# microsoft/tf2-gnn

Measured on AMD Instinct MI355X. Metric: edges/sec (fwd+bwd) RGCN H=320 L=4, PPI-shaped batch, 1/2/4/8 MI355X, higher is better.
Workload: dtype f32; 1 GPU; rmat30k: V=30000 E=900000 per GPU (one batch per rank, replicas) edge_types=4 D=320 H=320 layers=4 RGCN (PPI_RGCN.json stack settings), step = edge bucketing of the next batch (2nd stream, overlapped) + forward (training mode) + f...

## Files before the change

include/tfgnn.h:

```cpp
#ifndef TFGNN_H
#define TFGNN_H

#include <stddef.h>
#include <stdint.h>

#ifdef __cplusplus
extern "C" {
#endif

typedef enum {
  TFGNN_OK = 0,
  TFGNN_ERR_INVALID_ARGUMENT = -1,
  TFGNN_ERR_OUT_OF_RANGE = -2,
  TFGNN_ERR_HIP = -3,
  TFGNN_ERR_UNSUPPORTED = -4
} tfgnn_status;

typedef enum {
  TFGNN_ACT_NONE = 0,
  TFGNN_ACT_RELU = 1,
  TFGNN_ACT_TANH = 2,
  TFGNN_ACT_LEAKY_RELU = 3,
  TFGNN_ACT_ELU = 4,
  TFGNN_ACT_SELU = 5,
// ... 286 lines not shown
                        const float* d_fixed_inv_scale, void* stream);
int tfgnn_sp_split_cols(const float* d_src, int64_t ld, int64_t K, int64_t N, void* d_sp, int64_t ld_sp_bytes,
                        float* d_inv_scale, void* stream);
int tfgnn_sp_gemm_nt(int64_t M, int64_t N, int64_t K, const void* d_A_sp, int64_t lda_bytes, const float* d_a_inv_scale,
                     int a_scale_block, const void* d_B_sp, int64_t ldb_bytes, const float* d_b_inv_scale, float* d_C,
                     int64_t ldc, const float* d_bias, int act, int accumulate, const float* d_mul, int64_t ld_mul,
                     int act_of_saved, const float* d_saved, int64_t ld_saved, void* stream);
int tfgnn_sp_gemm_nt_sp(int64_t M, int64_t N, int64_t K, const void* d_A_sp, int64_t lda_bytes, const float* d_a_inv_scale,
                        int a_scale_block, const void* d_B_sp, int64_t ldb_bytes, const float* d_b_inv_scale, float* d_C,
                        int64_t ldc, const float* d_bias, int act, const float* d_mul, int64_t ld_mul, int act_of_saved,
                        const float* d_saved, int64_t ld_saved, void* d_out_sp, int64_t ld_out_sp_bytes,
                        float* d_out_inv_scale, void* stream);
int tfgnn_sp_gemm_nt_rows(int64_t M, int64_t N, int64_t K, const void* d_A_sp, int64_t lda_bytes, const float* d_a_inv_scale,
                          int a_scale_block, const int32_t* d_a_rows, const void* d_B_sp, int64_t ldb_bytes, const float* d_b_inv_scale,
                          float* d_C, int64_t ldc, const float* d_bias, int act, int accumulate, const float* d_mul, int64_t ld_mul,
                          int act_of_saved, const float* d_saved, int64_t ld_saved, float saved_scale, void* d_out_sp,
                          int64_t ld_out_sp_bytes, float* d_out_inv_scale, float dropout_rate, uint64_t dropout_seed,
                          const uint8_t* d_tile_kmask, const int32_t* d_row_map, void* stream);

int tfgnn_sp_gemm_nt_grouped(int64_t M, int64_t N, int64_t K, const void* d_A_sp, int64_t lda_bytes, const float* d_a_inv_scale,
                             int a_scale_block, const int32_t* d_a_rows, int64_t a_src_rows, const int32_t* d_tile_table,
                             int64_t num_tiles, int num_groups, const void* d_B_sp, int64_t ldb_bytes, int64_t b_group_stride_bytes,
                             const float* d_b_inv_scale, int64_t b_scale_group_stride, float* d_C, int64_t ldc, const float* d_bias,
                             int act, const float* d_mul, int64_t ld_mul, int act_of_saved, const float* d_saved, int64_t ld_saved,
                             void* d_out_sp, int64_t ld_out_sp_bytes, float* d_out_inv_scale, void* stream);
int tfgnn_sp_gather_rows(const void* d_src_sp, int64_t ld_src_bytes, const float* d_src_inv_scale, int scales_per_row,
                         const int32_t* d_index, int64_t rows, int64_t src_rows, int64_t cols, void* d_dst_sp, int64_t ld_dst_bytes,
                         float* d_dst_inv_scale, void* stream);

size_t tfgnn_sp_gemm_tn_wide_workspace_bytes(int64_t M, int64_t N, int64_t K, int64_t a_total_cols, int a_scale_block);
int tfgnn_sp_gemm_tn_wide(int64_t M, int64_t N, int64_t K, const void* d_A_sp, int64_t lda_bytes, int64_t a_first_col,
                          const float* d_a_inv_scale, int64_t a_total_cols, int a_scale_block, const void* d_B_sp,
                          int64_t ldb_bytes, int64_t b_first_col, const float* d_b_inv_scale, float* d_C, int64_t group_rows,
                          int64_t stride_group, int64_t stride_row, int64_t stride_col, int accumulate, void* d_workspace,
                          size_t workspace_bytes, void* stream);

size_t tfgnn_sp_gemm_tn_grouped_workspace_bytes(int64_t M, int64_t N, int64_t a_total_cols, int a_scale_block, int num_splits);
int tfgnn_sp_gemm_tn_grouped(int64_t M, int64_t N, const void* d_A_sp, int64_t lda_bytes, const float* d_a_inv_scale,
                             int64_t a_total_cols, int a_scale_block, const void* d_B_sp, int64_t ldb_bytes, const float* d_b_inv_scale,
                             int num_groups, const int32_t* d_group_split_offsets, int num_splits, const int32_t* d_split_table,
                             float* d_C, int64_t c_group_stride, int64_t stride_row, int64_t stride_col, void* d_workspace,
                             size_t workspace_bytes, void* stream);

int tfgnn_sp_gemm_nt_set_splitk_workspace(void* d_workspace, size_t bytes);
int tfgnn_sp_gemm_nt_splitk_status(int enable, int* timed_out, int64_t* split_launches);

int tfgnn_sp_gemm_nt_dropout(int64_t M, int64_t N, int64_t K, const void* d_A_sp, int64_t lda_bytes, const float* d_a_inv_scale,
                             int a_scale_block, const void* d_B_sp, int64_t ldb_bytes, const float* d_b_inv_scale, float* d_C,
                             int64_t ldc, const float* d_bias, int act, int accumulate, const float* d_mul, int64_t ld_mul,
                             int act_of_saved, const float* d_saved, int64_t ld_saved, float saved_scale, void* d_out_sp,
                             int64_t ld_out_sp_bytes, float* d_out_inv_scale, float dropout_rate, uint64_t dropout_seed,
                             const uint8_t* d_tile_kmask, const int32_t* d_row_map, void* stream);

typedef struct tfgnn_aux_job {
  int kind;
  unsigned num_blocks;
  unsigned char payload[248];
} tfgnn_aux_job;
int tfgnn_aux_launch(const tfgnn_aux_job* jobs, int num_jobs, void* stream);
int tfgnn_sp_split_rows_job(const float* d_src, int64_t ld, int64_t seg_len, int64_t seg_stride, int64_t rows, int64_t cols,
                            int scale_block, void* d_sp, int64_t ld_sp_bytes, float* d_inv_scale,
                            const float* d_fixed_inv_scale, tfgnn_aux_job* job);
int tfgnn_sp_split_cols_job(const float* d_src, int64_t ld, int64_t K, int64_t N, void* d_sp, int64_t ld_sp_bytes,
                            float* d_inv_scale, tfgnn_aux_job* job);
size_t tfgnn_sp_split_cols_two_pass_bytes(int64_t K, int64_t N);
int tfgnn_sp_split_cols_jobs(const float* d_src, int64_t ld, int64_t K, int64_t N, void* d_sp, int64_t ld_sp_bytes,
                             float* d_inv_scale, float* d_colmax_workspace, size_t workspace_bytes, tfgnn_aux_job* maxima_job,
                             tfgnn_aux_job* split_job);
int tfgnn_graph_gather_reduce_sp_deferred(const tfgnn_graph* graph, int view, const int32_t* d_col_override,
                                          const float* d_edge_weight, const float* d_row_scale, const float* d_in,
                                          int64_t ld_in, int width, void* d_out_sp, int64_t ld_out_sp_bytes,
                                          float* d_inv_scale, const float* d_fixed_inv_scale, void* d_workspace,
                                          size_t workspace_bytes, tfgnn_aux_job* combine_job, void* stream);

size_t tfgnn_sp_gemm_tn_workspace_bytes(int64_t M, int64_t N, int64_t K, int64_t a_total_cols, int a_scale_block);
int tfgnn_sp_spread_flag(int reset);
int tfgnn_sp_guard_repair(int on);
int tfgnn_sp_repair_stats(int64_t* out2, int reset);
int tfgnn_sp_gemm_tn(int64_t M, int64_t N, int64_t K, const void* d_A_sp, int64_t lda_bytes, int64_t a_first_col,
                     const float* d_a_inv_scale, int64_t a_total_cols, int a_scale_block, const void* d_B_sp,
                     int64_t ldb_bytes, int64_t b_first_col, const float* d_b_inv_scale, float* d_C, int64_t group_rows,
                     int64_t stride_group, int64_t stride_row, int64_t stride_col, int accumulate, void* d_workspace,
                     size_t workspace_bytes, void* stream);

int tfgnn_absmax(const float* d_x, int64_t n, float scale, float* d_out, void* stream);
int tfgnn_sp_inv_scale_from_bound(const float* d_bound, float* d_inv_scale, void* stream);

int tfgnn_graph_gather_dot_supported(int width, int ew_heads);
int tfgnn_graph_gather_reduce_dot(const tfgnn_graph* g, int view, const float* d_edge_weight, int ew_heads, const float* d_in,
                                  int64_t ld_in, int width, float* d_out, int64_t ld_out, const float* d_dot_rows, int64_t ld_dot,
                                  const int32_t* d_dot_pos, float* d_dot_out, void* d_workspace, size_t workspace_bytes,
                                  void* stream);

int tfgnn_graph_gather_reduce_sp(const tfgnn_graph* graph, int view, const int32_t* d_col_override,
                                 const float* d_edge_weight, const float* d_row_scale, const float* d_in, int64_t ld_in,
                                 int width, void* d_out_sp, int64_t ld_out_sp_bytes, float* d_inv_scale,
                                 const float* d_fixed_inv_scale, void* d_workspace, size_t workspace_bytes, void* stream);

int tfgnn_transpose_batched(const float* d_src, int64_t batch, int64_t rows, int64_t cols, float* d_dst,
                            void* stream);

size_t tfgnn_task_metrics_workspace_bytes(void);
int tfgnn_sigmoid_ce_metrics(const float* d_logits, int64_t ld_logits, const float* d_labels, int64_t ld_labels,
                             int64_t V, int64_t C, float* d_metrics, int64_t* d_counts, float* d_dlogits,
                             void* d_workspace, size_t workspace_bytes, void* stream);
int tfgnn_regression_metrics(const float* d_pred, const float* d_target, int64_t G, float* d_metrics,
                             float* d_dpred, void* d_workspace, size_t workspace_bytes, void* stream);
int tfgnn_binary_ce_metrics(const float* d_logits, const float* d_target, int64_t G, float* d_prob, float* d_metrics,
                            int64_t* d_counts, float* d_dlogits, void* d_workspace, size_t workspace_bytes,
                            void* stream);

size_t tfgnn_softmax_ce_workspace_bytes(void);
int tfgnn_softmax_ce_metrics(const float* d_logits, int64_t ld_logits, const float* d_labels, int64_t ld_labels,
                             const float* d_weights, int64_t ld_weights, int64_t V, int64_t C, float* d_metrics,
                             int64_t* d_counts, float* d_dlogits, int64_t ld_dlogits, int32_t* d_pred,
                             void* d_workspace, size_t workspace_bytes, void* stream);

size_t tfgnn_distmult_ce_workspace_bytes(void);
int tfgnn_distmult_ce_metrics(const float* d_H, int64_t ld_H, const float* d_R, const int32_t* d_triples, const float* d_labels,
                              int64_t ld_labels, const float* d_weights, int64_t ld_weights, int64_t V, int64_t T, int64_t N,
                              int64_t D, float* d_metrics, int64_t* d_counts, float* d_scores, float* d_gscore,
                              void* d_workspace, size_t workspace_bytes, void* stream);
size_t tfgnn_distmult_backward_workspace_bytes(int64_t N, int64_t D);
int tfgnn_distmult_backward(const float* d_H, int64_t ld_H, const float* d_R, const int32_t* d_triples, const float* d_gscore,
                            const int32_t* d_node_offsets, const int32_t* d_node_entries, const int32_t* d_rel_offsets,
                            const int32_t* d_rel_order, int64_t V, int64_t T, int64_t N, int64_t D, float* d_dH, int64_t ld_dH,
                            int accumulate, float* d_dR, void* d_workspace, size_t workspace_bytes, void* stream);
size_t tfgnn_distmult_rank_workspace_bytes(int64_t Q);
int tfgnn_distmult_rank(const float* d_H, int64_t ld_H, const float* d_R, const int32_t* d_queries, int64_t Q, int side,
                        const int32_t* d_filter_offsets, const int32_t* d_filter_ids, int64_t V, int64_t T, int64_t D,
                        int32_t* d_greater, int32_t* d_equal, void* d_workspace, size_t workspace_bytes, void* stream);
int tfgnn_link_launch_counts(int64_t* out_counts, int n);

typedef enum {
  TFGNN_MP_AGGREGATE_FIRST = 0
} tfgnn_mp_kind;

typedef struct tfgnn_mp_forward_args {
  size_t struct_size;
  int kind;
  const tfgnn_graph* graph;
  int view;
  const float* x;
  int64_t ldx;
  int in_dim, hidden_dim;
  const float* row_scale;
  const float* w;
  void* wt_sp;
  int64_t ld_wt_sp_bytes;
  float* wt_inv_scale;
  void* agg_sp;
  float* agg_inv_scale;
  const float* bias;
  int act;
  float dropout_rate;
  uint64_t dropout_seed;
  const uint8_t* tile_kmask;
  const int32_t* row_map;
  float* out;
  int64_t ld_out;
  void* out_sp;
  int64_t ld_out_sp_bytes;
  float* out_inv_scale;
  void* workspace;
  size_t workspace_bytes;
} tfgnn_mp_forward_args;
// ... 217 lines not shown
```

tf2_gnn_amd/_lib.py:

```python
from __future__ import annotations

import ctypes
from ctypes import POINTER, c_char_p, c_float, c_int, c_int32, c_int64, c_size_t, c_void_p
from pathlib import Path

LIB_PATH = Path(__file__).resolve().parent / "libtfgnn.so"

_SIGNATURES = [
    ("tfgnn_last_error", c_char_p, []),
    ("tfgnn_version", c_char_p, []),
    ("tfgnn_abi_version", c_int, []),
    ("tfgnn_gemm_gathered_supported", c_int, [c_int64, c_int64, c_int64, c_int64, c_int64]),
    ("tfgnn_launch_counts", c_int, [POINTER(c_int64), c_int]),
    ("tfgnn_sp_spread_flag", c_int, [c_int]),
    ("tfgnn_sp_guard_repair", c_int, [c_int]),
    ("tfgnn_sp_repair_stats", c_int, [POINTER(c_int64), c_int]),
    (
        "tfgnn_graph_create",
        c_int,
        [c_int, c_int64, POINTER(c_void_p), POINTER(c_int64), c_void_p, POINTER(c_void_p)],
    ),
    ("tfgnn_graph_destroy", c_int, [c_void_p]),
    (
        "tfgnn_graph_create_async",
# ... 215 lines not shown
         c_void_p, c_int64, c_int64, c_int64, c_void_p, c_size_t, c_void_p],
    ),
    ("tfgnn_sp_gemm_tn_wide_workspace_bytes", c_size_t, [c_int64, c_int64, c_int64, c_int64, c_int]),
    (
        "tfgnn_sp_gemm_tn_wide",
        c_int,
        [c_int64, c_int64, c_int64, c_void_p, c_int64, c_int64, c_void_p, c_int64, c_int, c_void_p, c_int64, c_int64, c_void_p,
         c_void_p, c_int64, c_int64, c_int64, c_int64, c_int, c_void_p, c_size_t, c_void_p],
    ),
    (
        "tfgnn_sp_gemm_tn",
        c_int,
        [c_int64, c_int64, c_int64, c_void_p, c_int64, c_int64, c_void_p, c_int64, c_int, c_void_p, c_int64, c_int64, c_void_p,
         c_void_p, c_int64, c_int64, c_int64, c_int64, c_int, c_void_p, c_size_t, c_void_p],
    ),
    ("tfgnn_absmax", c_int, [c_void_p, c_int64, c_float, c_void_p, c_void_p]),
    ("tfgnn_sp_inv_scale_from_bound", c_int, [c_void_p, c_void_p, c_void_p]),
    ("tfgnn_sp_bytes", c_size_t, [c_int64, c_int64]),
    (
        "tfgnn_sp_split_rows",
        c_int,
        [c_void_p, c_int64, c_int64, c_int64, c_int64, c_int64, c_int, c_void_p, c_int64, c_void_p, c_void_p, c_void_p],
    ),
    ("tfgnn_sp_split_cols", c_int, [c_void_p, c_int64, c_int64, c_int64, c_void_p, c_int64, c_void_p, c_void_p]),
    (
        "tfgnn_sp_gemm_nt",
        c_int,
        [c_int64, c_int64, c_int64, c_void_p, c_int64, c_void_p, c_int, c_void_p, c_int64, c_void_p, c_void_p, c_int64,
         c_void_p, c_int, c_int, c_void_p, c_int64, c_int, c_void_p, c_int64, c_void_p],
    ),
    (
        "tfgnn_sp_gemm_nt_sp",
        c_int,
        [c_int64, c_int64, c_int64, c_void_p, c_int64, c_void_p, c_int, c_void_p, c_int64, c_void_p, c_void_p, c_int64,
         c_void_p, c_int, c_void_p, c_int64, c_int, c_void_p, c_int64, c_void_p, c_int64, c_void_p, c_void_p],
    ),
    ("tfgnn_aux_launch", c_int, [c_void_p, c_int, c_void_p]),
    (
        "tfgnn_sp_split_rows_job",
        c_int,
        [c_void_p, c_int64, c_int64, c_int64, c_int64, c_int64, c_int, c_void_p, c_int64, c_void_p, c_void_p, c_void_p],
    ),
    ("tfgnn_sp_split_cols_job", c_int, [c_void_p, c_int64, c_int64, c_int64, c_void_p, c_int64, c_void_p, c_void_p]),
    ("tfgnn_sp_split_cols_two_pass_bytes", c_size_t, [c_int64, c_int64]),
    ("tfgnn_sp_split_cols_jobs", c_int, [c_void_p, c_int64, c_int64, c_int64, c_void_p, c_int64, c_void_p, c_void_p, c_size_t, c_void_p,
                                         c_void_p]),
    (
        "tfgnn_graph_gather_reduce_sp_deferred",
        c_int,
        [c_void_p, c_int, c_void_p, c_void_p, c_void_p, c_void_p, c_int64, c_int, c_void_p, c_int64, c_void_p, c_void_p, c_void_p,
         c_size_t, c_void_p, c_void_p],
    ),
    (
        "tfgnn_sp_gemm_nt_dropout",
        c_int,
        [c_int64, c_int64, c_int64, c_void_p, c_int64, c_void_p, c_int, c_void_p, c_int64, c_void_p, c_void_p, c_int64,
         c_void_p, c_int, c_int, c_void_p, c_int64, c_int, c_void_p, c_int64, c_float, c_void_p, c_int64, c_void_p, c_float,
         ctypes.c_uint64, c_void_p, c_void_p, c_void_p],
    ),
    (
        "tfgnn_sp_gemm_nt_grouped",
        c_int,
        [c_int64, c_int64, c_int64, c_void_p, c_int64, c_void_p, c_int, c_void_p, c_int64, c_void_p, c_int64, c_int, c_void_p, c_int64,
         c_int64, c_void_p, c_int64, c_void_p, c_int64, c_void_p, c_int, c_void_p, c_int64, c_int, c_void_p, c_int64, c_void_p, c_int64,
         c_void_p, c_void_p],
    ),
    ("tfgnn_sp_gather_rows", c_int, [c_void_p, c_int64, c_void_p, c_int, c_void_p, c_int64, c_int64, c_int64, c_void_p, c_int64,
                                     c_void_p, c_void_p]),
    (
        "tfgnn_sp_gemm_nt_rows",
        c_int,
        [c_int64, c_int64, c_int64, c_void_p, c_int64, c_void_p, c_int, c_void_p, c_void_p, c_int64, c_void_p, c_void_p, c_int64,
         c_void_p, c_int, c_int, c_void_p, c_int64, c_int, c_void_p, c_int64, c_float, c_void_p, c_int64, c_void_p, c_float,
         ctypes.c_uint64, c_void_p, c_void_p, c_void_p],
    ),
]

_SIGNATURES += [
    ("tfgnn_mp_forward", c_int, [c_void_p, c_void_p]),
    ("tfgnn_mp_backward", c_int, [c_void_p, c_void_p]),
]

_SIGNATURES += [
    ("tfgnn_pool_workspace_bytes", c_size_t, [c_int64, c_int64, c_int, c_int, c_int]),
    ("tfgnn_pool_forward", c_int, [c_void_p, c_void_p]),
    ("tfgnn_pool_backward", c_int, [c_void_p, c_void_p]),
    ("tfgnn_pool_launch_counts", c_int, [POINTER(c_int64), c_int]),
]
POOL_SOFTMAX, POOL_SIGMOID, POOL_NONE, POOL_AVERAGE = range(4)
POOL_CHUNK_NODES = 128

_SIGNATURES += [
    ("tfgnn_optimizer_workspace_bytes", c_size_t, [c_void_p, c_int, c_int]),
    ("tfgnn_optimizer_apply", c_int, [c_void_p, c_int, c_void_p, c_void_p]),
    ("tfgnn_optimizer_iterations_get", c_int, [c_void_p, c_void_p, c_void_p]),
    ("tfgnn_optimizer_iterations_set", c_int, [c_void_p, c_int64, c_void_p]),
    ("tfgnn_optimizer_launch_count", c_int64, []),
]

_SIGNATURES += [
    ("tfgnn_batch_assemble", c_int, [c_void_p, c_void_p]),
    ("tfgnn_batch_assemble_launch_counts", c_int, [POINTER(c_int64), c_int]),
]
BATCH_MAX_EDGE_TYPES = 48
BATCH_MAX_COLUMNS = 8
BATCH_MAX_NODE_COLUMNS = 4

_SIGNATURES += [
    ("tfgnn_distmult_ce_workspace_bytes", c_size_t, []),
    (
        "tfgnn_distmult_ce_metrics",
        c_int,
        [c_void_p, c_int64, c_void_p, c_void_p, c_void_p, c_int64, c_void_p, c_int64, c_int64, c_int64, c_int64, c_int64, c_void_p,
         c_void_p, c_void_p, c_void_p, c_void_p, c_size_t, c_void_p],
    ),
    ("tfgnn_distmult_backward_workspace_bytes", c_size_t, [c_int64, c_int64]),
    (
        "tfgnn_distmult_backward",
        c_int,
        [c_void_p, c_int64, c_void_p, c_void_p, c_void_p, c_void_p, c_void_p, c_void_p, c_void_p, c_int64, c_int64, c_int64, c_int64,
         c_void_p, c_int64, c_int, c_void_p, c_void_p, c_size_t, c_void_p],
    ),
    ("tfgnn_distmult_rank_workspace_bytes", c_size_t, [c_int64]),
    (
        "tfgnn_distmult_rank",
        c_int,
        [c_void_p, c_int64, c_void_p, c_void_p, c_int64, c_int, c_void_p, c_void_p, c_int64, c_int64, c_int64, c_void_p, c_void_p,
         c_void_p, c_size_t, c_void_p],
    ),
    ("tfgnn_link_launch_counts", c_int, [POINTER(c_int64), c_int]),
]
LINK_CHUNK = 256

_SIGNATURES += [
    ("tfgnn_neighbor_sample_workspace_bytes", c_size_t, [c_int64, c_int, c_int64]),
    ("tfgnn_neighbor_sample", c_int, [c_void_p, c_void_p]),
    ("tfgnn_gather_node_rows", c_int, [c_void_p, c_void_p]),
    ("tfgnn_sample_launch_counts", c_int, [POINTER(c_int64), c_int]),
]
SAMPLE_MAX_HOPS = 8
SAMPLE_META_STATUS, SAMPLE_META_NODES, SAMPLE_META_EDGES = 0, 1, 2
SAMPLE_NODE_OVERFLOW, SAMPLE_EDGE_OVERFLOW, SAMPLE_REPEATED_SEED, SAMPLE_BAD_SEED, SAMPLE_BAD_STORE = 1, 2, 4, 8, 16


def sample_meta_words(num_edge_types: int, num_hops: int) -> int:
    return 2 + num_edge_types + num_hops + 2


EXPORTED_SYMBOLS = [s[0] for s in _SIGNATURES]
ABI_VERSION = 5


class AuxJob(ctypes.Structure):

    _fields_ = [("kind", c_int), ("num_blocks", ctypes.c_uint), ("payload", ctypes.c_ubyte * 248)]


class MpForwardArgs(ctypes.Structure):

    _fields_ = [
        ("struct_size", ctypes.c_size_t), ("kind", c_int), ("graph", c_void_p), ("view", c_int), ("x", c_void_p), ("ldx", c_int64),
        ("in_dim", c_int), ("hidden_dim", c_int), ("row_scale", c_void_p), ("w", c_void_p), ("wt_sp", c_void_p),
        ("ld_wt_sp_bytes", c_int64), ("wt_inv_scale", c_void_p), ("agg_sp", c_void_p), ("agg_inv_scale", c_void_p), ("bias", c_void_p),
        ("act", c_int), ("dropout_rate", ctypes.c_float), ("dropout_seed", ctypes.c_uint64), ("tile_kmask", c_void_p),
        ("row_map", c_void_p), ("out", c_void_p), ("ld_out", c_int64), ("out_sp", c_void_p), ("ld_out_sp_bytes", c_int64),
        ("out_inv_scale", c_void_p), ("workspace", c_void_p), ("workspace_bytes", ctypes.c_size_t),
    ]


class MpBackwardArgs(ctypes.Structure):

    _fields_ = [
        ("struct_size", ctypes.c_size_t), ("kind", c_int), ("graph", c_void_p), ("d_pre", c_void_p), ("ld_d_pre", c_int64),
        ("in_dim", c_int), ("hidden_dim", c_int), ("edge_weight", c_void_p), ("w", c_void_p), ("wh_sp", c_void_p),
        ("ld_wh_sp_bytes", c_int64), ("wh_inv_scale", c_void_p), ("g_sp", c_void_p), ("g_inv_scale", c_void_p), ("dx", c_void_p),
        ("ld_dx", c_int64), ("accumulate", c_int), ("mul", c_void_p), ("ld_mul", c_int64), ("act_of_saved", c_int), ("saved", c_void_p),
        ("ld_saved", c_int64), ("saved_scale", ctypes.c_float), ("dropout_rate", ctypes.c_float), ("dropout_seed", ctypes.c_uint64),
        ("dx_sp", c_void_p), ("ld_dx_sp_bytes", c_int64), ("dx_inv_scale", c_void_p), ("tile_kmask", c_void_p), ("a_rows", c_void_p),
        ("row_map", c_void_p), ("dw", c_void_p), ("x_sp", c_void_p), ("ld_x_sp_bytes", c_int64), ("x_inv_scale", c_void_p),
        ("tn_workspace", c_void_p), ("tn_workspace_bytes", ctypes.c_size_t), ("workspace", c_void_p),
        ("workspace_bytes", ctypes.c_size_t),
    ]


class PoolForwardArgs(ctypes.Structure):

    _fields_ = [
        ("struct_size", ctypes.c_size_t), ("kind", c_int), ("V", c_int64), ("G", c_int64), ("GD", c_int), ("heads", c_int),
        ("ptr", c_void_p), ("T", c_void_p), ("ldT", c_int64), ("S", c_void_p), ("ldS", c_int64), ("lo", c_float), ("hi", c_float),
        ("out", c_void_p), ("w", c_void_p), ("ldw", c_int64), ("workspace", c_void_p), ("workspace_bytes", ctypes.c_size_t),
    ]


class PoolBackwardArgs(ctypes.Structure):

    _fields_ = [
        ("struct_size", ctypes.c_size_t), ("kind", c_int), ("V", c_int64), ("G", c_int64), ("GD", c_int), ("heads", c_int),
        ("ptr", c_void_p), ("ids", c_void_p), ("dOut", c_void_p), ("T", c_void_p), ("ldT", c_int64), ("w", c_void_p),
        ("ldw", c_int64), ("lo", c_float), ("hi", c_float), ("dT", c_void_p), ("lddT", c_int64), ("dS", c_void_p),
        ("lddS", c_int64), ("workspace", c_void_p), ("workspace_bytes", ctypes.c_size_t),
    ]


class BatchAssembleArgs(ctypes.Structure):

    _fields_ = [
        ("struct_size", ctypes.c_size_t), ("num_edge_types", c_int), ("num_columns", c_int), ("num_graphs", c_int64),
        ("store_nodes", c_int64), ("feature_dim", c_int64), ("node_ptr", c_void_p), ("features", c_void_p), ("edge_ptr", c_void_p),
        ("edges", c_void_p), ("columns", c_void_p), ("order_len", c_int64), ("order", c_void_p), ("pos_node_ptr", c_void_p),
        ("pos_edge_ptr", c_void_p), ("p0", c_int64), ("p1", c_int64), ("num_nodes", c_int64), ("num_edges", c_void_p),
        ("node_features", c_void_p), ("node_to_graph_map", c_void_p), ("adjacency_lists", c_void_p), ("column_out", c_void_p),
        ("bad_flag", c_void_p), ("num_node_columns", c_int), ("node_column_widths", c_void_p), ("node_columns", c_void_p),
        ("node_column_out", c_void_p),
    ]


class NeighborSampleArgs(ctypes.Structure):

    _fields_ = [
        ("struct_size", ctypes.c_size_t), ("num_edge_types", c_int), ("num_hops", c_int), ("num_nodes", c_int64),
        ("in_ptr", c_void_p), ("in_src", c_void_p), ("store_edges", c_void_p), ("fanouts", c_void_p), ("seed", ctypes.c_uint64),
        ("num_seeds", c_int64), ("seeds", c_void_p), ("node_capacity", c_int64), ("edge_capacity", c_void_p), ("nodes", c_void_p),
        ("adjacency_lists", c_void_p), ("meta", c_void_p), ("workspace", c_void_p), ("workspace_bytes", ctypes.c_size_t),
    ]


class GatherNodeRowsArgs(ctypes.Structure):

    _fields_ = [
        ("struct_size", ctypes.c_size_t), ("store_nodes", c_int64), ("num_rows", c_int64), ("num_seeds", c_int64), ("nodes", c_void_p),
        ("feature_dim", c_int64), ("features", c_void_p), ("node_features", c_void_p), ("num_node_columns", c_int),
        ("node_column_widths", c_void_p), ("node_columns", c_void_p), ("node_column_out", c_void_p), ("seed_only", c_void_p),
        ("bad_flag", c_void_p),
    ]


class OptConfig(ctypes.Structure):

# ... 48 lines not shown
```

tf2_gnn_amd/csrc/gemm_sp.hip:

```cpp
#include <algorithm>
#include <cstdlib>

#include <type_traits>

#include "aux_jobs.hpp"
#include "common.hpp"
#include "gemm_sp.hpp"
#include "sp16.hpp"
#include "tn_repair.hpp"

namespace tfgnn {

template <int I, int N, class F>
__device__ __forceinline__ void static_for(F&& f) {
  if constexpr (I < N) {
    f(std::integral_constant<int, I>{});
    static_for<I + 1, N>(f);
  }
}

typedef _Float16 half8 __attribute__((ext_vector_type(8)));
typedef _Float16 half2v __attribute__((ext_vector_type(2)));
typedef float floatx16 __attribute__((ext_vector_type(16)));
typedef unsigned int uint4v __attribute__((ext_vector_type(4)));
typedef unsigned int uint2v __attribute__((ext_vector_type(2)));
typedef __attribute__((address_space(3))) void lds_void;

constexpr int SP_BM = 128;
constexpr int SP_NT = 256;

struct SpArgs {
  int64_t M, N, K;
  const uint8_t* A;
  int64_t lda;
  const float* a_inv;
  int64_t a_inv_ld;
  int a_nblk;
  int a_blk_steps;
  const uint8_t* B;
  int64_t ldb;
  const float* b_inv;
  float* C;
  int64_t ldc;
  const float* bias;
  int act;
  int accumulate;
  const float* mul;
  int64_t ld_mul;
  const float* saved;
  int64_t ld_saved;
  int dact;
  unsigned n_tiles;
  uint8_t* out_sp;
  int64_t ld_out_sp;
  float* out_inv;
  int drop_on;
  int64_t drop_ld;
  DropoutKey drop;
  float saved_scale;
  const uint8_t* tile_kmask;
  const int32_t* row_map;
  const int32_t* a_rows;
  int64_t a_src_rows;
  const int32_t* tile_table;
  int64_t group_stride_b;
  int64_t group_stride_scale;
  int ksplit;
  float* ws_partial;
  unsigned* ws_flags;
  int* ws_timeout;
  unsigned xcd_per, xcd_total;
};

__global__ void __launch_bounds__(256) sp_split_rows_kernel(const float* __restrict__ src, int64_t ld, int64_t seg_len,
                                                            int64_t seg_stride, int64_t R, int64_t C, int sb,
                                                            uint8_t* __restrict__ dst, int64_t ld_dst, float* __restrict__ inv,
                                                            const float* __restrict__ fixed_inv) {
  sp_split_rows_body(src, ld, seg_len, seg_stride, R, C, sb, dst, ld_dst, inv, fixed_inv, blockIdx.x);
}

template <int LPR>
__global__ void __launch_bounds__(256) sp_split_rows_narrow_kernel(const float* __restrict__ src, int64_t ld, int64_t R,
                                                                   uint8_t* __restrict__ dst, int64_t ld_dst, float* __restrict__ inv) {
  constexpr int RPB = 256 / LPR;
  const int sub = threadIdx.x % LPR;
  for (int64_t r = (int64_t)blockIdx.x * RPB + threadIdx.x / LPR; r < R; r += (int64_t)gridDim.x * RPB) {
    const float4 v = *reinterpret_cast<const float4*>(src + r * ld + sub * 4);
    float mx = fmaxf(fmaxf(fabsf(v.x), fabsf(v.y)), fmaxf(fabsf(v.z), fabsf(v.w)));
#pragma unroll
    for (int o = LPR / 2; o; o >>= 1) mx = fmaxf(mx, __shfl_xor(mx, o, 64));
    float iv;
    const float sc = sp_scale_for_max(mx, &iv);
    if (inv && sub == 0) inv[r] = iv;
    sp_store4(dst + r * ld_dst, sub * 4, v, sc);
  }
}

__global__ void __launch_bounds__(256) sp_absmax_kernel(const float* __restrict__ x, int64_t n, float scale, float* out) {
  float mx = 0.f;
  const int64_t n4 = n >> 2;
  for (int64_t i = (int64_t)blockIdx.x * blockDim.x + threadIdx.x; i < n4; i += (int64_t)gridDim.x * blockDim.x) {
    const float4 v = reinterpret_cast<const float4*>(x)[i];
    mx = fmaxf(mx, fmaxf(fmaxf(fabsf(v.x), fabsf(v.y)), fmaxf(fabsf(v.z), fabsf(v.w))));
  }
  if (blockIdx.x == 0 && threadIdx.x < (n & 3)) mx = fmaxf(mx, fabsf(x[(n4 << 2) + threadIdx.x]));
#pragma unroll
  for (int o = 32; o; o >>= 1) mx = fmaxf(mx, __shfl_xor(mx, o, 64));
  __shared__ float wmax[4];
  if ((threadIdx.x & 63) == 0) wmax[threadIdx.x >> 6] = mx;
  __syncthreads();
  if (threadIdx.x == 0)
    atomicMax(reinterpret_cast<unsigned*>(out), __float_as_uint(fmaxf(fmaxf(wmax[0], wmax[1]), fmaxf(wmax[2], wmax[3])) * scale));
}

__global__ void sp_inv_scale_kernel(const float* bound, float* inv) {
  float iv;
  (void)sp_scale_for_max(fabsf(bound[0]), &iv);
  inv[0] = iv;
}

__global__ void __launch_bounds__(256) sp_split_cols_kernel(const float* __restrict__ src, int64_t ld, int64_t K, int64_t N,
                                                            uint8_t* __restrict__ dst, int64_t ld_dst, float* __restrict__ inv) {
  sp_split_cols_body(src, ld, K, N, dst, ld_dst, inv, blockIdx.x, blockIdx.y, gridDim.y);
}

template <int TNW>
constexpr int sp_nt_tm = TNW == 5 ? 1 : 2;

template <int TNW, int TM = 2>
struct SpGeo {
  static constexpr int BN = 64 * TNW;
  static constexpr int ROWS = SP_BM + BN;
  static constexpr int STG = ROWS * 64;
  static constexpr int NW = 8 / TM;
  static constexpr int NT = 64 * NW;
  static constexpr int ND_A = 8 / NW;
  static constexpr int ND_B = 4 * TNW / NW;
  static constexpr int ND = ND_A + ND_B;
  static constexpr bool PAIR = TM == 1;
  static constexpr bool SHARED = (4 * TNW) % NW != 0;
  static constexpr int NI = PAIR ? 2 * ND + (SHARED ? 1 : 0) : ND;
  static_assert(!SHARED || (PAIR && 4 * TNW - NW * ND_B == NW / 2), "left-over units go to wave pairs");
  static constexpr int PATCH_ROWS = 16 * TM;
  static constexpr int PATCH_LD = 32 * TNW + 4;
  static constexpr int NST_MAX = TNW == 2 ? 4 : 6;
  static constexpr int NST = (163840 / STG) < NST_MAX ? (163840 / STG) : NST_MAX;
  static constexpr int UNR = NST % 2 == 0 ? NST : 2 * NST;
  static constexpr int VMW = PAIR ? NI : (NST - 3) * ND;
  static constexpr int LDS_BYTES = NST * STG;
  static_assert(NST >= 4 && VMW < 64, "ring depth");
  static_assert(!PAIR || NST % 2 == 1, "pair issue fills the ring NST - 1 steps ahead, two steps at a time");
  static_assert(NW * PATCH_ROWS * PATCH_LD * 4 + TM * NW * 32 * 4 <= LDS_BYTES, "epilogue patch and row maxima must fit the ring");
};

template <int TNW, int TM>
struct SpLoop {
// ... 99 lines not shown
    if constexpr (I < N) {
      read_one<I, SET, ST>();
      read_all<I + 1, N, SET, ST>();
    }
  }

  const float* a_inv;
  int a_nblk, a_blk_steps;
  int64_t a_row[TM];
  float a_rmax[TM];
  half2v afac[TM];
  template <int SET>
  __device__ __forceinline__ void scale_frags(int step) {
    asm volatile("s_waitcnt lgkmcnt(0)" ::: "memory");
    const int lstep = step + (int)step0;
    if (lstep % a_blk_steps == 0 || step == 0) {
      const int q = step < nsteps ? lstep / a_blk_steps : 0;
      const int b = bsteps ? (int)((blkmap >> (4u * (unsigned)q)) & 15u) : q;
      if (step < nsteps && b < a_nblk) {
#pragma unroll
        for (int t = 0; t < TM; ++t) {
          const _Float16 f = (_Float16)(a_inv[a_row[t] * a_nblk + b] / a_rmax[t]);
          afac[t] = half2v{f, f};
        }
      }
    }
#pragma unroll
    for (int t = 0; t < TM; ++t)
#pragma unroll
      for (int p = 0; p < 2; ++p) {
        half2v* v = reinterpret_cast<half2v*>(&fa[SET][t][p]);
#pragma unroll
        for (int j = 0; j < 4; ++j) v[j] = v[j] * afac[t];
      }
  }

  static constexpr int NR = 2 * TM + 2 * TNW;
  static constexpr int NM = 3 * TM * TNW;
  static constexpr int DMA0 = NM - G::NI < NR ? NM - G::NI : NR;
  static_assert(DMA0 >= 0 && DMA0 + G::NI <= NM, "issue pattern");
  template <int S, int I, bool ABLK>
  __device__ __forceinline__ void step_items(int sbase) {
    if constexpr (I < NM) {
      mfma_one<I, (S & 1)>();
      if constexpr (I < NR) read_one<I, ((S + 1) & 1), ((S + 1) % G::NST)>();
      if constexpr (G::PAIR) {
        if constexpr ((S & 1) == 0 && I >= DMA0 && I < DMA0 + G::NI) dma_pair<I - DMA0, S>();
      } else {
        if constexpr (I >= DMA0 && I < DMA0 + G::NI) dma_one<I - DMA0, ((S + G::NST - 1) % G::NST)>(sbase + S + G::NST - 1);
      }
      if constexpr (ABLK && I == NM - 1) scale_frags<((S + 1) & 1)>(sbase + S + 1);
      step_items<S, I + 1, ABLK>(sbase);
    }
  }
  template <int S, bool ABLK>
  __device__ __forceinline__ void step(int sbase) {
    if constexpr (G::PAIR && (S & 1) == 0) pair_offsets(sbase + S);
    step_items<S, 0, ABLK>(sbase);
    asm volatile("s_waitcnt vmcnt(%0) lgkmcnt(0)" ::"n"(G::VMW) : "memory");
    __builtin_amdgcn_s_barrier();
  }
  template <int S, bool ABLK>
  __device__ __forceinline__ void steps(int sbase) {
    if constexpr (S < G::UNR) {
      if (sbase + S < nsteps) step<S, ABLK>(sbase);
      steps<S + 1, ABLK>(sbase);
    }
  }
  template <int J>
  __device__ __forceinline__ void dma_prologue() {
    if constexpr (G::PAIR) {
      if constexpr (2 * J < G::NST - 1) {
        pair_offsets(-(G::NST - 1) + 2 * J);
        dma_pair_all<0, (G::NST + 1 + 2 * J) % G::UNR>();
        dma_prologue<J + 1>();
      }
    } else if constexpr (J < G::NST - 1) {
      dma_all<0, G::ND, J>(J);
      dma_prologue<J + 1>();
    }
  }
};

template <int TNW, bool ABLK, bool GRAD, bool OUT_SP = false>
__global__ void __launch_bounds__((SpGeo<TNW, sp_nt_tm<TNW>>::NT), (TNW == 2 ? 2 : 1)) gemm_sp_nt_kernel(SpArgs g) {
  constexpr int TM = sp_nt_tm<TNW>;
  using G = SpGeo<TNW, TM>;
  constexpr int WR = 32 * TM;
  extern __shared__ __attribute__((aligned(16))) uint8_t lds[];
  const int tid = threadIdx.x;
  const int lane = tid & 63;
  const int wave = __builtin_amdgcn_readfirstlane(tid >> 6);
  const int wm = wave >> 1, wn = wave & 1;
  unsigned bid = blockIdx.x;
  if (g.xcd_per) {
    bid = (blockIdx.x & 7u) * g.xcd_per + (blockIdx.x >> 3);
    if (bid >= g.xcd_total) return;
  }
  int split = 0;
  int S = g.ksplit;
  if (S > 1) {
    const unsigned nt_all = gridDim.x / (unsigned)S;
    if (bid < nt_all * (unsigned)(S - 1)) {
      split = 1 + (int)(bid / nt_all);
      bid -= (unsigned)(split - 1) * nt_all;
    } else {
      bid -= nt_all * (unsigned)(S - 1);
    }
  }
  const unsigned tile_n = bid % g.n_tiles;
  const unsigned tile_m = bid / g.n_tiles;
  int64_t row0 = (int64_t)tile_m * SP_BM, m_end = g.M;
  int64_t grp = 0;
  if (g.tile_table) {
    const int32_t* e = g.tile_table + 4 * (int64_t)tile_m;
    row0 = __builtin_amdgcn_readfirstlane(e[0]);
    m_end = row0 + __builtin_amdgcn_readfirstlane(e[1]);
    grp = __builtin_amdgcn_readfirstlane(e[2]);
  }
  const int64_t col0 = (int64_t)tile_n * G::BN;
  int nsteps = (int)(g.K >> 4);
  unsigned blkmap = 0, bsteps = 0;
  if (g.tile_kmask) {
    unsigned m = __builtin_amdgcn_readfirstlane((int)g.tile_kmask[tile_m]) & ((1u << g.a_nblk) - 1u);
    if (!m) m = 1u;
    int n = 0;
    for (int b = 0; b < g.a_nblk; ++b)
      if (m & (1u << b)) blkmap |= (unsigned)b << (4 * n++);
    bsteps = (unsigned)g.a_blk_steps;
    nsteps = n * g.a_blk_steps;
  }
  unsigned step0 = 0;
  if (S > 1) {
    const int P = (int)(g.K >> 4);
    const int per = (P + S - 1) / S;
    const int p0 = split * per, p1 = p0 + per < P ? p0 + per : P;
    if (!bsteps) {
      step0 = (unsigned)p0;
      nsteps = p1 > p0 ? p1 - p0 : 0;
    } else {
      int first = -1, cnt = 0;
      const int nb = nsteps / (int)bsteps;
      for (int q = 0; q < nb; ++q) {
        const int b = (int)((blkmap >> (4u * (unsigned)q)) & 15u);
        const int lo = p0 > b * (int)bsteps ? p0 : b * (int)bsteps;
        const int hi = p1 < (b + 1) * (int)bsteps ? p1 : (b + 1) * (int)bsteps;
        if (hi > lo) {
          if (first < 0) first = q * (int)bsteps + (lo - b * (int)bsteps);
          cnt += hi - lo;
        }
      }
      step0 = first < 0 ? 0u : (unsigned)first;
      nsteps = cnt;
    }
  }

  const int64_t rows_a = m_end - row0 < SP_BM ? m_end - row0 : SP_BM;
  const int64_t rows_b = g.N - col0 < G::BN ? g.N - col0 : G::BN;
  auto make_rsrc = [](const uint8_t* p, int64_t bytes) {
    const uint64_t a = (uint64_t)(uintptr_t)p;
    return uint4v{(unsigned)__builtin_amdgcn_readfirstlane((int)(unsigned)a),
                  (unsigned)__builtin_amdgcn_readfirstlane((int)(unsigned)((a >> 32) & 0xffffu)),
                  (unsigned)__builtin_amdgcn_readfirstlane((int)bytes), 0x00020000u};
  };
  const uint4v rs_a = g.a_rows ? make_rsrc(g.A, g.a_src_rows * g.lda) : make_rsrc(g.A + row0 * g.lda, rows_a * g.lda);
  const uint4v rs_b = make_rsrc(g.B + grp * g.group_stride_b + col0 * g.ldb, rows_b * g.ldb);
  half8 r_fa[2][TM][2];
  half8 r_fb[2][TNW][2];
  floatx16 r_acc[TM][TNW];
  unsigned r_aa[G::NST][2], r_ba[G::NST][2], r_va[G::ND_A], r_vb[SpLoop<TNW, TM>::NVB];
  SpLoop<TNW, TM> L(r_fa, r_fb, r_acc, r_aa, r_ba, r_va, r_vb);
  L.rs_a = rs_a;
  L.rs_b = rs_b;
  const unsigned lds_base = (unsigned)(uintptr_t)(lds_void*)lds;
  L.m0_a = __builtin_amdgcn_readfirstlane(lds_base + wave * G::ND_A * 1024);
  L.m0_b = __builtin_amdgcn_readfirstlane(lds_base + wave * G::ND_B * 1024);
  L.m0_s = __builtin_amdgcn_readfirstlane(lds_base + SP_BM * 64 + (G::NW * G::ND_B + (wave >> 1)) * 1024);
  L.half_s = wave & 1;
  L.nsteps = nsteps;
  L.blkmap = blkmap;
  L.step0 = step0;
  L.bsteps = bsteps;
  L.brecip = bsteps ? (65536u + bsteps - 1u) / bsteps : 0u;
  const int drow = lane >> 2;
  const int dq = (lane & 3) ^ ((drow >> 2) & 3);
// ... 766 lines not shown
          fa[j] = 0.f;
          anz[j] = false;
          if (j < nb && k < krows) {
            const float ia = g.inv_a[(k0 + k) * g.a_nblk + blk_first + j];
            fa[j] = ia * fref[j];
            anz[j] = ia > 1.2e-38f;
            if (anz[j]) famax = fmaxf(famax, fa[j]);
          }
        }
        const bool bnz = k < krows && ib > 1.2e-38f;
        const float fbv = k < krows ? ib * frefb : 0.f;
        float fb2 = fbv, up = 1.f;
        if (bnz && famax > 0.f) {
          const unsigned ex = (__float_as_uint(famax * fbv) >> 23) & 0xffu;
          if (ex > 0u && ex <= 127u) {
            const unsigned tb = (127u - ex) >> 1;
            fb2 = __uint_as_float((127u - tb) << 23);
            up = fbv * __uint_as_float((127u + tb) << 23);
          }
        }
        ftab[(k >> 4) * FH + 64 + (k & 15)] = (_Float16)fb2;
        wide |= bnz && famax > 0.f && fb2 < 2.384185791015625e-07f;
#pragma unroll
        for (int j = 0; j < 4; ++j) {
          const float f = anz[j] ? fa[j] * up : 0.f;
          ftab[(k >> 4) * FH + j * 16 + (k & 15)] = (_Float16)f;
          wide |= anz[j] && bnz && f < 2.384185791015625e-07f;
        }
      } else {
#pragma unroll
        for (int j = 0; j < 4; ++j) {
          float f = 0.f, ia = 0.f;
          if (j < nb && k < krows) {
            ia = g.inv_a[(k0 + k) * g.a_nblk + blk_first + j];
            f = sp_row_holds(ia, ib) ? ia * ib * fref[j] : 0.f;
          }
          ftab[(k >> 4) * FH + j * 16 + (k & 15)] = (_Float16)f;
          wide |= sp_row_too_small(f, ia, ib);
        }
      }
    }
    if (g.spread_flag && __any(wide) && lane == 0) g.spread_flag[split * g.trip_stride] = 1;
  }
  L.wait_landed();
  __builtin_amdgcn_s_barrier();
  __builtin_amdgcn_sched_barrier(0);
  L.template load_factors<0>(0);
  L.template read_all<0, NR, 0, 0>();
  L.template scale_all<0, (BSC ? NR : 4), 0>();
  __builtin_amdgcn_sched_barrier(0);
  for (int s = 0; s < nsteps; s += G::UNR) L.template steps<0>(s);
  asm volatile("s_waitcnt vmcnt(0)\n\ts_nop 15\n\ts_nop 15" ::: "memory");
  __builtin_amdgcn_s_barrier();

  float* patch = reinterpret_cast<float*>(lds) + wave * 32 * G::PATCH_LD;
  float* __restrict__ part = g.partial + (int64_t)split * g.M * g.N;
  const int64_t wcol0 = col0 + wn * 32 * TNW;
  constexpr int C4 = 8 * TNW;
  constexpr int NIT = 32 * C4 / 64;
  auto store_tile = [&](auto t_c) {
    constexpr int t = decltype(t_c)::value;
#pragma unroll
    for (int c = 0; c < TNW; ++c)
#pragma unroll
      for (int r = 0; r < 16; ++r) {
        const int prow = (r & 3) + 8 * (r >> 2) + 4 * kg;
        patch[prow * G::PATCH_LD + c * 32 + fi] = L.acc[t][c][r];
      }
    asm volatile("s_waitcnt lgkmcnt(0)" ::: "memory");
    const int64_t wrow0 = row0 + wm * 64 + t * 32;
#pragma unroll
    for (int it = 0; it < NIT; ++it) {
      const int idx = lane + it * 64;
      const int pr = idx / C4, c4 = idx - pr * C4;
      const float4 v = *reinterpret_cast<const float4*>(patch + pr * G::PATCH_LD + c4 * 4);
      *reinterpret_cast<float4*>(part + (wrow0 + pr) * g.N + wcol0 + c4 * 4) = v;
    }
    asm volatile("s_waitcnt lgkmcnt(0)" ::: "memory");
  };
  store_tile(std::integral_constant<int, 0>{});
  store_tile(std::integral_constant<int, 1>{});
}

struct TnReduceArgs {
  const float* partial;
  int splits;
  int64_t M, N;
  const float* ref;
  int64_t a_col0;
  int a_sb;
  float* C;
  int64_t group_rows, stride_group, stride_row, stride_col;
  int accumulate;
  int64_t slab;
  int ref_ld;
};

__device__ __forceinline__ void sp_tn_reduce_body(const TnReduceArgs& a, unsigned block, unsigned nblocks) {
  const int64_t total = a.M * a.N;
  for (int64_t i = (int64_t)block * 256 + threadIdx.x; i < total; i += (int64_t)nblocks * 256) {
    const int64_t m = i / a.N, n = i - m * a.N;
    const int64_t blk = (a.a_col0 + m) / a.a_sb;
    float s = 0.f;
    int z = 0;
    if (a.ref_ld > 0) {
      for (; z + 8 <= a.splits; z += 8) {
        float v[8], r[8];
#pragma unroll
        for (int u = 0; u < 8; ++u) {
          v[u] = a.partial[(int64_t)(z + u) * a.slab + i];
          r[u] = a.ref[(int64_t)(z + u) * a.ref_ld + blk];
        }
#pragma unroll
        for (int u = 0; u < 8; ++u) s += v[u] * r[u];
      }
      for (; z < a.splits; ++z) s += a.partial[(int64_t)z * a.slab + i] * a.ref[(int64_t)z * a.ref_ld + blk];
    } else {
      for (; z + 8 <= a.splits; z += 8) {
        float v[8];
#pragma unroll
        for (int u = 0; u < 8; ++u) v[u] = a.partial[(int64_t)(z + u) * a.slab + i];
#pragma unroll
        for (int u = 0; u < 8; ++u) s += v[u];
      }
      for (; z < a.splits; ++z) s += a.partial[(int64_t)z * a.slab + i];
      s *= a.ref[blk];
    }
    const int64_t gi = m / a.group_rows, mi = m - gi * a.group_rows;
    float* dst = a.C + gi * a.stride_group + mi * a.stride_row + n * a.stride_col;
    *dst = a.accumulate ? *dst + s : s;
  }
}

__global__ void __launch_bounds__(256) sp_tn_reduce_kernel(TnReduceArgs a) { sp_tn_reduce_body(a, blockIdx.x, gridDim.x); }
__global__ void __launch_bounds__(256) sp_tn_reduce_grouped_kernel(TnReduceArgs a, const int32_t* __restrict__ split_off,
                                                                   int64_t c_group_stride) {
  const int gq = blockIdx.y;
  const int s0 = split_off[gq], s1 = split_off[gq + 1];
  a.partial += (int64_t)s0 * a.slab;
  a.ref += (int64_t)s0 * a.ref_ld;
  a.splits = s1 - s0;
  a.C += (int64_t)gq * c_group_stride;
  sp_tn_reduce_body(a, blockIdx.x, gridDim.x);
}

static int sp_tn_splits(int64_t M, int64_t N, int64_t K, int bn) {
  const int64_t tiles = (M / SP_BM) * (N / bn);
  const int64_t steps = (K + 15) / 16;
  int64_t splits = std::max<int64_t>(1, std::min<int64_t>(250 / std::max<int64_t>(tiles, 1), steps / 16));
  return (int)std::max<int64_t>(1, splits);
}

template <int TNW>
static void launch_sp_nt(const SpArgs& g_in, dim3 grid, hipStream_t s) {
  using G = SpGeo<TNW, sp_nt_tm<TNW>>;
  SpArgs g = g_in;
  g.xcd_per = g.xcd_total = 0;
  static const bool xcd_order = [] { const char* e = getenv("TFGNN_SP_NT_XCD"); return !(e && atoi(e) == 0); }();
  if (xcd_order && g.n_tiles > 1 && g.ksplit <= 1 && grid.y == 1 && grid.z == 1 && grid.x >= 16) {
    g.xcd_total = grid.x;
    g.xcd_per = (grid.x + 7u) / 8u;
    grid.x = g.xcd_per * 8u;
  }
  const bool ablk = g.a_inv && g.a_nblk > 1;
  const bool grad = g.mul || g.saved;
  count_launch(TFGNN_KFAM_SP_NT);
  using Kernel = void (*)(SpArgs);
  static const Kernel kernels[2][2][2] = {
      {{gemm_sp_nt_kernel<TNW, false, false, false>, gemm_sp_nt_kernel<TNW, false, false, true>},
       {gemm_sp_nt_kernel<TNW, false, true, false>, gemm_sp_nt_kernel<TNW, false, true, true>}},
      {{gemm_sp_nt_kernel<TNW, true, false, false>, gemm_sp_nt_kernel<TNW, true, false, true>},
       {gemm_sp_nt_kernel<TNW, true, true, false>, gemm_sp_nt_kernel<TNW, true, true, true>}}};
  static bool attr_set[2][2][2] = {};
  const bool out_sp = g.out_sp != nullptr;
  const Kernel kernel = kernels[ablk][grad][out_sp];
  if (!attr_set[ablk][grad][out_sp]) {
    (void)hipFuncSetAttribute((const void*)kernel, hipFuncAttributeMaxDynamicSharedMemorySize, G::LDS_BYTES);
    attr_set[ablk][grad][out_sp] = true;
  }
  hipLaunchKernelGGL(kernel, grid, dim3(G::NT), G::LDS_BYTES, s, g);
}

constexpr size_t kSplitkFlagBytes = 65536;
struct SplitkWorkspace {
  void* base = nullptr;
  size_t bytes = 0;
  bool enabled = true;
  long long split_launches = 0;
  long long timeouts = 0;
  int device = -1;
  hipStream_t last_stream = nullptr;
  bool used = false;
  int* timeout_host = nullptr;
  int* timeout_dev = nullptr;
};
static SplitkWorkspace g_splitk;

static bool stream_is_capturing(hipStream_t s) {
  hipStreamCaptureStatus st = hipStreamCaptureStatusNone;
  if (hipStreamIsCapturing(s, &st) != hipSuccess) {
    (void)hipGetLastError();
    return false;
  }
  return st != hipStreamCaptureStatusNone;
}

static int splitk_admit(hipStream_t s) {
  if (!(g_splitk.enabled && g_splitk.base)) return 0;
  if (g_splitk.timeout_host && __atomic_load_n(g_splitk.timeout_host, __ATOMIC_RELAXED)) {
    ++g_splitk.timeouts;
    __atomic_store_n(g_splitk.timeout_host, 0, __ATOMIC_RELAXED);
    (void)hipDeviceSynchronize();
    (void)hipMemset(g_splitk.base, 0, kSplitkFlagBytes);
    set_error("tfgnn_sp_gemm_nt: a reducer of an earlier K-split product gave up waiting for its producers - that product's "
              "result is incomplete; the workspace flags were cleared (tfgnn_sp_gemm_nt_splitk_status reports the count)");
    return -1;
  }
  int dev = -1;
  if (hipGetDevice(&dev) != hipSuccess || dev != g_splitk.device) {
    (void)hipGetLastError();
    return 0;
  }
  if (g_splitk.used && s != g_splitk.last_stream) {
    if (stream_is_capturing(g_splitk.last_stream)) return 0;
    if (!stream_is_capturing(s)) {
      if (hipStreamSynchronize(g_splitk.last_stream) != hipSuccess) {
        (void)hipGetLastError();
        return 0;
      }
    }
  }
  g_splitk.last_stream = s;
  g_splitk.used = true;
  return 1;
}

static int sp_colmax_parts(int64_t K) { return (int)std::max<int64_t>(1, std::min<int64_t>(256, K / 160)); }

static int sp_tile_width(int64_t N) { return N % 320 == 0 ? 320 : (N % 256 == 0 ? 256 : (N % 128 == 0 ? 128 : 0)); }

static int* g_spread_host = nullptr;
static int* g_spread_dev = nullptr;
static int* sp_spread_flag_device() {
  if (!g_spread_host) {
    int* h = nullptr;
    if (hipHostMalloc((void**)&h, 64, hipHostMallocMapped) != hipSuccess) {
      (void)hipGetLastError();
      return nullptr;
    }
    *h = 0;
    void* d = nullptr;
    if (hipHostGetDevicePointer(&d, h, 0) != hipSuccess) {
      (void)hipGetLastError();
      (void)hipHostFree(h);
      return nullptr;
    }
    g_spread_host = h;
    g_spread_dev = (int*)d;
  }
  return g_spread_dev;
}

constexpr int kSpTnMaxRanges = 512;
static_assert(kSpTnMaxRanges == kTnRepairGroupedMaxRanges, "the repair tail holds one trip word per K range of a launch");

struct TnLayout {
  size_t ref, ref_split, slabs, tail, total;
  int64_t f_ld;
};
static TnLayout sp_tn_layout(int64_t Mp, int64_t N, int64_t nblk, int64_t kpad, bool factor_pass, int64_t ranges, size_t tail_bytes) {
  TnLayout l;
  const int pass_floats = factor_pass ? 1 + SP_TN_MAXCHUNKS : 0;
  l.ref = factor_pass ? ((size_t)nblk * kpad * 2 + 255) & ~(size_t)255 : 0;
  l.ref_split = l.ref + (size_t)nblk * pass_floats * 4;
  l.slabs = l.ref + (((size_t)nblk * (pass_floats + kSpTnMaxRanges) * 4 + 255) & ~(size_t)255);
  l.tail = l.slabs + (size_t)ranges * (size_t)Mp * (size_t)N * 4;
  l.total = l.tail + tail_bytes;
  l.f_ld = factor_pass ? kpad : 0;
  return l;
}

enum class TnForm { FactorPass, OneFactor, TwoFactor };

template <int TNW, bool FIK, bool BSC>
static void launch_sp_tn_form(const SpTnArgs& g, dim3 grid, hipStream_t s) {
  constexpr int lds = SpGeoTN<TNW, FIK, BSC>::LDS_BYTES;
  [[maybe_unused]] static const hipError_t attr_set =
      hipFuncSetAttribute((const void*)gemm_sp_tn_kernel<TNW, FIK, BSC>, hipFuncAttributeMaxDynamicSharedMemorySize, lds);
  hipLaunchKernelGGL((gemm_sp_tn_kernel<TNW, FIK, BSC>), grid, dim3(SP_NT), lds, s, g);
}

template <int TNW>
static void launch_sp_tn(TnForm form, const SpTnArgs& g, dim3 grid, hipStream_t s) {
  count_launch(TFGNN_KFAM_SP_TN);
  if (form == TnForm::TwoFactor) launch_sp_tn_form<TNW, true, true>(g, grid, s);
  else if (form == TnForm::OneFactor) launch_sp_tn_form<TNW, true, false>(g, grid, s);
  else launch_sp_tn_form<TNW, false, false>(g, grid, s);
}

struct TnLaunch {
  int64_t M, N, K;
  const uint8_t *A, *B;
  int64_t lda, ldb;
  const float *inv_a, *inv_b;
  int a_sb, a_nblk;
  int64_t a_col0;
  int splits;
  int64_t k_chunk;
  const int32_t* split_table;
  TnForm form;
  uint8_t* ws;
  TnLayout lay;
  bool repair;
  int trip_stride;
  float* C;
  int64_t group_rows, stride_group, stride_row, stride_col;
  int accumulate;
  int num_groups;
  const int32_t* group_split_offsets;
  int64_t c_group_stride;
};

static int sp_tn_enqueue(const TnLaunch& t, hipStream_t s) {
  const int bn = sp_tile_width(t.N);
  const int64_t Mp = ceil_div(t.M, SP_BM) * SP_BM;
  const bool armed = t.repair && t.splits > 0, per_split = t.form != TnForm::FactorPass;
  float* ref = (float*)(t.ws + t.lay.ref);
  float* ref_split = (float*)(t.ws + t.lay.ref_split);
  int* guard_word = sp_spread_flag_device();
  if (armed) {
    guard_word = (int*)(t.ws + t.lay.tail);
    if (int rc = tn_repair_begin(guard_word, t.trip_stride ? kTnRepairGroupedTailBytes : sizeof(int), s)) return rc;
  }
  SpTnArgs g{};
  g.M = Mp; g.N = t.N; g.K = t.K;
  g.A = t.A; g.lda = t.lda;
  g.B = t.B; g.ldb = t.ldb;
  g.F = t.lay.f_ld ? (const _Float16*)t.ws : nullptr; g.f_ld = t.lay.f_ld;
  g.a_sb = t.a_sb; g.a_col0 = t.a_col0; g.a_nblk = t.a_nblk;
  g.inv_a = t.inv_a; g.inv_b = t.inv_b; g.ref_split = ref_split; g.spread_flag = guard_word;
  g.trip_stride = t.trip_stride;
  g.partial = (float*)(t.ws + t.lay.slabs);
  g.k_chunk = t.k_chunk;
  g.split_table = t.split_table;
  g.n_tiles = (unsigned)(t.N / bn);
  g.tiles = (unsigned)((Mp / SP_BM) * g.n_tiles);
  g.splits = (unsigned)t.splits;
  g.per_xcd = (g.tiles * g.splits + 7) / 8;
  if (t.form == TnForm::FactorPass) {
    const int fch = sp_tn_fchunks(t.K);
    float* slice_max = nullptr;
    if (fch > SP_TN_FCHUNKS) {
      slice_max = ref + t.a_nblk;
      hipLaunchKernelGGL(sp_tn_slice_max_kernel, dim3((unsigned)t.a_nblk * fch), dim3(1024), 0, s, t.inv_a, (int64_t)t.a_nblk, t.inv_b,
                         (int64_t)1, t.K, slice_max, fch);
    }
    hipLaunchKernelGGL(sp_tn_factors_kernel, dim3((unsigned)t.a_nblk * fch), dim3(1024), 0, s, t.inv_a, (int64_t)t.a_nblk, t.inv_b,
                       (int64_t)1, t.K, (_Float16*)t.ws, t.lay.f_ld, ref, guard_word, fch, (const float*)slice_max);
    TFGNN_LAUNCH_CHECK();
  }
  if (t.splits > 0) {
    const dim3 grid(8 * g.per_xcd);
    if (bn == 320) launch_sp_tn<5>(t.form, g, grid, s);
    else if (bn == 256) launch_sp_tn<4>(t.form, g, grid, s);
    else launch_sp_tn<2>(t.form, g, grid, s);
    TFGNN_LAUNCH_CHECK();
  }
  if (armed) {
    TnRepairArgs rp{};
    rp.M = t.M; rp.N = t.N; rp.K = t.K; rp.A = t.A; rp.lda = t.lda; rp.B = t.B; rp.ldb = t.ldb;
    rp.inv_a = t.inv_a; rp.inv_b = t.inv_b; rp.a_sb = t.a_sb; rp.a_col0 = t.a_col0; rp.a_nblk = t.a_nblk;
    rp.partial = g.partial; rp.slab = Mp * t.N; rp.splits = t.splits;
    rp.k_chunk = t.split_table ? 0 : t.k_chunk; rp.split_table = t.split_table;
    rp.ref = per_split ? ref_split : ref; rp.ref_per_split = per_split ? 1 : 0; rp.trip = guard_word;
    if (int rc = tn_repair_enqueue(rp, s)) return rc;
  }
  TnReduceArgs ra{};
  ra.partial = g.partial; ra.M = t.M; ra.N = t.N; ra.ref = per_split ? ref_split : ref; ra.a_col0 = t.a_col0; ra.a_sb = t.a_sb;
  ra.ref_ld = per_split ? t.a_nblk : 0;
  ra.splits = t.group_split_offsets ? 0 : t.splits;
  ra.C = t.C; ra.group_rows = t.group_rows; ra.stride_group = t.stride_group; ra.stride_row = t.stride_row; ra.stride_col = t.stride_col;
  ra.accumulate = t.accumulate; ra.slab = Mp * t.N;
  const int64_t rblocks = ceil_div(t.M * t.N, 256);
  if (t.group_split_offsets) {
    hipLaunchKernelGGL(sp_tn_reduce_grouped_kernel, dim3((unsigned)std::min<int64_t>(rblocks, 512), (unsigned)t.num_groups), dim3(256), 0, s,
                       ra, t.group_split_offsets, t.c_group_stride);
  } else {
    hipLaunchKernelGGL(sp_tn_reduce_kernel, dim3((unsigned)std::min<int64_t>(rblocks, 2048)), dim3(256), 0, s, ra);
  }
  TFGNN_LAUNCH_CHECK();
  return TFGNN_OK;
}

static int sp_tn_check_operands(const char* who, int64_t M, int64_t N, const void* d_A_sp, int64_t lda_bytes, int64_t a_first_col,
                                int64_t a_total_cols, int a_scale_block, const void* d_B_sp, int64_t ldb_bytes, int64_t b_first_col,
                                bool column_ranges) {
  if (!sp_tile_width(N) || M % 16 || a_scale_block < 32) {
    set_error("%s: M = %lld must be a multiple of 16, N = %lld of 128, scale blocks of A >= 32 columns", who, (long long)M, (long long)N);
    return TFGNN_ERR_UNSUPPORTED;
  }
  TFGNN_REQUIRE(lda_bytes % 64 == 0 && ldb_bytes % 64 == 0 && (uintptr_t)d_A_sp % 64 == 0 && (uintptr_t)d_B_sp % 64 == 0 &&
                    a_first_col % 16 == 0 && b_first_col % 16 == 0 && a_first_col >= 0 && b_first_col >= 0 &&
                    lda_bytes >= (a_first_col + M) * 4 && ldb_bytes >= (b_first_col + N) * 4 && a_total_cols >= a_first_col + M &&
                    a_total_cols % a_scale_block == 0,
                "%s: SP16 operands must be 64-byte aligned%s", who,
                column_ranges ? ", first columns multiples of 16, rows wide enough" : " with rows wide enough");
  return TFGNN_OK;
}

static int sp_tn_check_workspace(const char* who, const void* d_workspace, size_t workspace_bytes, size_t need) {
  TFGNN_REQUIRE(d_workspace && workspace_bytes >= need && (uintptr_t)d_workspace % 256 == 0,
                "%s: workspace too small or unaligned (need %zu bytes)", who, need);
  return TFGNN_OK;
}

struct NtShape {
  int bn;
  int a_scale_block;
  bool a_uniform;
  int64_t a_src_rows;
  int64_t group_stride_b;
  int drop_on;
  DropoutKey drop;
  int64_t tiles;
};

static int sp_nt_check(const NtCall& c, NtShape* d) {
  const int64_t M = c.M, N = c.N, K = c.K;
  TFGNN_REQUIRE(c.A && c.B && (c.C || c.out_sp), "tfgnn_sp_gemm_nt: null pointer");
  d->a_src_rows = (!c.a_rows || c.a_src_rows <= 0) ? M : c.a_src_rows;
  TFGNN_REQUIRE(!c.a_rows || d->a_src_rows * c.lda_bytes < (1ll << 32) - 65536, "tfgnn_sp_gemm_nt_rows: the operand read through a row index must be below 4 GB");
  TFGNN_REQUIRE(!c.tile_table || (c.num_tiles_m > 0 && c.num_groups >= 1 && !c.tile_kmask && !c.row_map),
                "tfgnn_sp_gemm_nt_grouped: a tile table needs its tile count and excludes the tile mask / row map");
  TFGNN_REQUIRE(c.dropout_rate >= 0.f && c.dropout_rate < 1.f, "tfgnn_sp_gemm_nt: dropout rate must be in [0, 1), got %f", (double)c.dropout_rate);
  TFGNN_REQUIRE(M > 0 && N > 0 && K > 0 && K % 16 == 0, "tfgnn_sp_gemm_nt: K must be a positive multiple of 16");
  d->bn = sp_tile_width(N);
  if (!d->bn) {
    set_error("tfgnn_sp_gemm_nt: N = %lld is not a multiple of 128", (long long)N);
    return TFGNN_ERR_UNSUPPORTED;
  }
  TFGNN_REQUIRE(c.lda_bytes % 64 == 0 && c.ldb_bytes % 64 == 0 && c.lda_bytes >= K * 4 && c.ldb_bytes >= K * 4 &&
                    (uintptr_t)c.A % 64 == 0 && (uintptr_t)c.B % 64 == 0,
                "tfgnn_sp_gemm_nt: SP16 operands must be 64-byte aligned with leading dimensions >= 4 K bytes");
  TFGNN_REQUIRE((!c.C || (c.ldc % 4 == 0 && (uintptr_t)c.C % 16 == 0)) && (!c.bias || (uintptr_t)c.bias % 16 == 0) &&
                    (!c.b_inv_scale || (uintptr_t)c.b_inv_scale % 16 == 0) && (!c.mul || (c.ld_mul % 4 == 0 && (uintptr_t)c.mul % 16 == 0)) &&
                    (!c.saved || (c.ld_saved % 4 == 0 && (uintptr_t)c.saved % 16 == 0)),
                "tfgnn_sp_gemm_nt: C / bias / scale / factor operands must be 16-byte aligned with ld %% 4 == 0");
  TFGNN_REQUIRE(128 * c.lda_bytes < (1ll << 31) && 320 * c.ldb_bytes < (1ll << 31), "tfgnn_sp_gemm_nt: K too large");
  d->a_uniform = c.a_scale_block < 0;
  d->a_scale_block = (c.a_scale_block <= 0 || c.a_scale_block >= K) ? (int)K : c.a_scale_block;
  TFGNN_REQUIRE(d->a_scale_block % 16 == 0 && K % d->a_scale_block == 0, "tfgnn_sp_gemm_nt: a_scale_block must divide K and be a multiple of 16");
  if (c.tile_kmask) {
    const int a_nblk = (int)(K / d->a_scale_block), a_blk_steps = d->a_scale_block / 16;
    TFGNN_REQUIRE(a_nblk >= 1 && a_nblk <= 8 && a_blk_steps <= 64 && a_blk_steps * a_nblk == (int)(K >> 4) && c.a_inv_scale &&
                      !d->a_uniform,
                  "tfgnn_sp_gemm_nt: the tile mask needs 1..8 scale blocks of A (of at most 1024 columns) that tile K");
  }
  d->group_stride_b = c.b_group_stride_bytes >= 0 ? c.b_group_stride_bytes : N * c.ldb_bytes;
  TFGNN_REQUIRE(d->group_stride_b % 64 == 0, "tfgnn_sp_gemm_nt_grouped: group stride of B must be a multiple of 64 bytes");
  d->drop_on = c.dropout_rate > 0.f ? (c.dropout_seed == ~0ull ? 2 : 1) : 0;
  if (d->drop_on == 2)
    TFGNN_REQUIRE(c.saved && c.act_of_saved == TFGNN_ACT_RELU, "tfgnn_sp_gemm_nt_dropout: the mask-from-saved form needs a relu saved tensor");
  d->drop = dropout_key(c.dropout_seed, c.dropout_rate);
  TFGNN_REQUIRE(c.dropout_rate <= 0.f || d->drop.epoch, "tfgnn_sp_gemm_nt_dropout: no device memory for this device's epoch word");
  if (c.out_sp) {
    TFGNN_REQUIRE(!c.accumulate && c.out_inv_scale, "tfgnn_sp_gemm_nt_sp: the split result needs no accumulation and an inverse-scale array");
    TFGNN_REQUIRE(c.ld_out_sp_bytes >= N * 4 && c.ld_out_sp_bytes % 64 == 0 && (uintptr_t)c.out_sp % 64 == 0,
                  "tfgnn_sp_gemm_nt_sp: SP16 result rows must be 64-byte aligned and at least 4 N bytes");
  }
  d->tiles = (c.tile_table ? c.num_tiles_m : ceil_div(M, SP_BM)) * (unsigned)(N / d->bn);
  TFGNN_REQUIRE(d->tiles <= 0x7fffffff, "tfgnn_sp_gemm_nt: too many tiles");
  return TFGNN_OK;
}

static SpArgs sp_nt_args(const NtCall& c, const NtShape& d) {
  SpArgs g{};
  g.M = c.M; g.N = c.N; g.K = c.K;
  g.A = (const uint8_t*)c.A; g.lda = c.lda_bytes; g.a_inv = c.a_inv_scale;
  g.a_nblk = (int)(c.K / d.a_scale_block);
  g.a_inv_ld = d.a_uniform ? 0 : g.a_nblk;
  g.a_blk_steps = d.a_scale_block / 16;
  g.B = (const uint8_t*)c.B; g.ldb = c.ldb_bytes; g.b_inv = c.b_inv_scale;
  g.C = c.C; g.ldc = c.ldc; g.bias = c.bias; g.act = c.act; g.accumulate = c.accumulate;
  g.mul = c.mul; g.ld_mul = c.ld_mul; g.saved = c.saved; g.ld_saved = c.ld_saved; g.dact = c.act_of_saved;
  g.saved_scale = c.saved_scale;
  g.tile_kmask = c.tile_kmask;
  g.row_map = c.row_map;
  g.a_rows = c.a_rows;
  g.a_src_rows = d.a_src_rows;
  g.tile_table = c.tile_table;
  g.group_stride_b = d.group_stride_b;
  g.group_stride_scale = c.b_scale_group_stride >= 0 ? c.b_scale_group_stride : c.N;
  g.drop_on = d.drop_on;
  g.drop_ld = c.N;
  g.drop = d.drop;
  g.n_tiles = (unsigned)(c.N / d.bn);
  if (c.out_sp) {
    g.out_sp = (uint8_t*)c.out_sp; g.ld_out_sp = c.ld_out_sp_bytes; g.out_inv = c.out_inv_scale;
  }
  g.ksplit = 1;
  return g;
}

constexpr int kSplitkMaxSplits = 4;
constexpr int64_t kSplitkMinSteps = 15;
constexpr int64_t kSplitkMaxWorkgroups = 232;
constexpr int64_t kSplitkMaxTiles = 112;

static int sp_nt_plan_splitk(SpArgs& g, const NtShape& d, hipStream_t s) {
  const int64_t steps = g.K >> 4;
  int S = (int)std::min<int64_t>(kSplitkMaxSplits, steps / kSplitkMinSteps);
  while (S > 1 && d.tiles * S > kSplitkMaxWorkgroups) --S;
  if (!(g_splitk.enabled && g_splitk.base && S > 1 && d.tiles <= kSplitkMaxTiles && !g.tile_table)) return TFGNN_OK;
  const size_t slab = (size_t)SP_BM * d.bn * 4;
  const size_t need = kSplitkFlagBytes + (size_t)d.tiles * (S - 1) * slab;
  const int admit = (need <= g_splitk.bytes && (size_t)d.tiles * (S - 1) * 4 <= kSplitkFlagBytes) ? splitk_admit(s) : 0;
  if (admit < 0) return TFGNN_ERR_HIP;
  if (admit > 0) {
    g.ksplit = S;
    ++g_splitk.split_launches;
    g.ws_flags = (unsigned*)g_splitk.base;
    g.ws_partial = (float*)((char*)g_splitk.base + kSplitkFlagBytes);
    g.ws_timeout = g_splitk.timeout_dev;
  }
  return TFGNN_OK;
}

int sp_nt_enqueue(const NtCall& c, hipStream_t s) {
  NtShape d;
  int rc = sp_nt_check(c, &d);
  if (rc) return rc;
  SpArgs g = sp_nt_args(c, d);
  rc = sp_nt_plan_splitk(g, d, s);
  if (rc) return rc;
  const dim3 grid((unsigned)(d.tiles * g.ksplit));
  if (d.bn == 320) launch_sp_nt<5>(g, grid, s);
  else if (d.bn == 256) launch_sp_nt<4>(g, grid, s);
  else launch_sp_nt<2>(g, grid, s);
  TFGNN_LAUNCH_CHECK();
  return TFGNN_OK;
}

}

using namespace tfgnn;

extern "C" {

size_t tfgnn_sp_bytes(int64_t rows, int64_t cols) { return (size_t)rows * (size_t)cols * 4; }

int tfgnn_sp_spread_flag(int reset) {
  if (!g_spread_host) return 0;
  const int v = __atomic_load_n(g_spread_host, __ATOMIC_RELAXED);
  if (reset) __atomic_store_n(g_spread_host, 0, __ATOMIC_RELAXED);
  return v;
}

int tfgnn_sp_split_rows(const float* d_src, int64_t ld, int64_t seg_len, int64_t seg_stride, int64_t rows, int64_t cols,
                        int scale_block, void* d_sp, int64_t ld_sp_bytes, float* d_inv_scale,
                        const float* d_fixed_inv_scale, void* stream) {
  TFGNN_REQUIRE(d_src && d_sp, "tfgnn_sp_split_rows: null pointer");
  TFGNN_REQUIRE(rows >= 0 && cols > 0 && cols % 16 == 0, "tfgnn_sp_split_rows: cols must be a positive multiple of 16");
  if (scale_block <= 0) scale_block = (int)cols;
  if (seg_len <= 0) { seg_len = cols; seg_stride = 0; }
  TFGNN_REQUIRE(scale_block % 16 == 0 && cols % scale_block == 0, "tfgnn_sp_split_rows: scale_block must divide cols and be a multiple of 16");
  TFGNN_REQUIRE(seg_len % 4 == 0 && cols % seg_len == 0 && ld % 4 == 0 && seg_stride % 4 == 0 && (uintptr_t)d_src % 16 == 0,
                "tfgnn_sp_split_rows: source must be 16-byte aligned with segment length / strides multiples of 4");
  TFGNN_REQUIRE(ld_sp_bytes >= cols * 4 && ld_sp_bytes % 64 == 0 && (uintptr_t)d_sp % 64 == 0, "tfgnn_sp_split_rows: bad SP16 leading dimension / alignment");
  if (rows == 0) return TFGNN_OK;
  if (!d_fixed_inv_scale && scale_block == cols && (seg_len <= 0 || seg_len >= cols) && rows >= 4096 &&
      (cols == 64 || cols == 128 || cols == 256)) {
    const unsigned rpb = (unsigned)(256 / (cols / 4));
    const unsigned grid = (unsigned)std::min<int64_t>(ceil_div(rows, rpb), 256 * 32);
    hipStream_t s = (hipStream_t)stream;
    if (cols == 64) hipLaunchKernelGGL(sp_split_rows_narrow_kernel<16>, dim3(grid), dim3(256), 0, s, d_src, ld, rows, (uint8_t*)d_sp, ld_sp_bytes, d_inv_scale);
    else if (cols == 128) hipLaunchKernelGGL(sp_split_rows_narrow_kernel<32>, dim3(grid), dim3(256), 0, s, d_src, ld, rows, (uint8_t*)d_sp, ld_sp_bytes, d_inv_scale);
    else hipLaunchKernelGGL(sp_split_rows_narrow_kernel<64>, dim3(grid), dim3(256), 0, s, d_src, ld, rows, (uint8_t*)d_sp, ld_sp_bytes, d_inv_scale);
    TFGNN_LAUNCH_CHECK();
    return TFGNN_OK;
  }
  const int64_t items = rows * (cols / scale_block);
  hipLaunchKernelGGL(sp_split_rows_kernel, dim3((unsigned)ceil_div(items, 4)), dim3(256), 0, (hipStream_t)stream, d_src, ld,
                     seg_len, seg_stride, rows, cols, scale_block, (uint8_t*)d_sp, ld_sp_bytes, d_inv_scale, d_fixed_inv_scale);
  TFGNN_LAUNCH_CHECK();
  return TFGNN_OK;
}

int tfgnn_sp_split_cols(const float* d_src, int64_t ld, int64_t K, int64_t N, void* d_sp, int64_t ld_sp_bytes,
                        float* d_inv_scale, void* stream) {
  TFGNN_REQUIRE(d_src && d_sp, "tfgnn_sp_split_cols: null pointer");
  TFGNN_REQUIRE(K > 0 && N > 0 && K % 16 == 0 && N % 4 == 0 && ld % 4 == 0 && (uintptr_t)d_src % 16 == 0,
                "tfgnn_sp_split_cols: K must be a multiple of 16, N and ld multiples of 4");
  TFGNN_REQUIRE(ld_sp_bytes >= K * 4 && ld_sp_bytes % 64 == 0 && (uintptr_t)d_sp % 64 == 0, "tfgnn_sp_split_cols: bad SP16 leading dimension / alignment");
  hipLaunchKernelGGL(sp_split_cols_kernel, dim3((unsigned)ceil_div(N, 16), (unsigned)std::max<int64_t>(1, std::min<int64_t>(8, K / 128))), dim3(256), 0, (hipStream_t)stream, d_src, ld, K, N,
                     (uint8_t*)d_sp, ld_sp_bytes, d_inv_scale);
  TFGNN_LAUNCH_CHECK();
  return TFGNN_OK;
}

int tfgnn_sp_gemm_nt_set_splitk_workspace(void* d_workspace, size_t bytes) {
  TFGNN_HIP_CHECK(hipDeviceSynchronize());
  if (!d_workspace || bytes <= kSplitkFlagBytes) {
    g_splitk.base = nullptr;
    g_splitk.bytes = 0;
    return TFGNN_OK;
  }
  TFGNN_REQUIRE((uintptr_t)d_workspace % 256 == 0, "tfgnn_sp_gemm_nt_set_splitk_workspace: the workspace must be 256-byte aligned");
  if (!g_splitk.timeout_host) {
    int* h = nullptr;
    void* d = nullptr;
    if (hipHostMalloc((void**)&h, 64, hipHostMallocMapped) == hipSuccess && hipHostGetDevicePointer(&d, h, 0) == hipSuccess) {
      *h = 0;
      g_splitk.timeout_host = h;
      g_splitk.timeout_dev = (int*)d;
    } else {
      (void)hipGetLastError();
    }
  }
  TFGNN_HIP_CHECK(hipMemset(d_workspace, 0, kSplitkFlagBytes));
  TFGNN_HIP_CHECK(hipGetDevice(&g_splitk.device));
  g_splitk.base = d_workspace;
// ... 47 lines not shown
                             int a_scale_block, const void* d_B_sp, int64_t ldb_bytes, const float* d_b_inv_scale, float* d_C,
                             int64_t ldc, const float* d_bias, int act, int accumulate, const float* d_mul, int64_t ld_mul,
                             int act_of_saved, const float* d_saved, int64_t ld_saved, float saved_scale, void* d_out_sp,
                             int64_t ld_out_sp_bytes, float* d_out_inv_scale, float dropout_rate, uint64_t dropout_seed,
                             const uint8_t* d_tile_kmask, const int32_t* d_row_map, void* stream) {
  NtCall c;
  c.M = M; c.N = N; c.K = K;
  c.A = d_A_sp; c.lda_bytes = lda_bytes; c.a_inv_scale = d_a_inv_scale; c.a_scale_block = a_scale_block;
  c.B = d_B_sp; c.ldb_bytes = ldb_bytes; c.b_inv_scale = d_b_inv_scale;
  c.C = d_C; c.ldc = ldc; c.accumulate = accumulate;
  c.out_sp = d_out_sp; c.ld_out_sp_bytes = ld_out_sp_bytes; c.out_inv_scale = d_out_inv_scale;
  c.bias = d_bias; c.act = act;
  c.mul = d_mul; c.ld_mul = ld_mul; c.act_of_saved = act_of_saved; c.saved = d_saved; c.ld_saved = ld_saved;
  c.saved_scale = saved_scale; c.dropout_rate = dropout_rate; c.dropout_seed = dropout_seed;
  c.tile_kmask = d_tile_kmask; c.row_map = d_row_map;
  return sp_nt_enqueue(c, (hipStream_t)stream);
}

int tfgnn_sp_gemm_nt_rows(int64_t M, int64_t N, int64_t K, const void* d_A_sp, int64_t lda_bytes, const float* d_a_inv_scale,
                          int a_scale_block, const int32_t* d_a_rows, const void* d_B_sp, int64_t ldb_bytes, const float* d_b_inv_scale,
                          float* d_C, int64_t ldc, const float* d_bias, int act, int accumulate, const float* d_mul, int64_t ld_mul,
                          int act_of_saved, const float* d_saved, int64_t ld_saved, float saved_scale, void* d_out_sp,
                          int64_t ld_out_sp_bytes, float* d_out_inv_scale, float dropout_rate, uint64_t dropout_seed,
                          const uint8_t* d_tile_kmask, const int32_t* d_row_map, void* stream) {
  NtCall c;
  c.M = M; c.N = N; c.K = K;
  c.A = d_A_sp; c.lda_bytes = lda_bytes; c.a_inv_scale = d_a_inv_scale; c.a_scale_block = a_scale_block; c.a_rows = d_a_rows;
  c.B = d_B_sp; c.ldb_bytes = ldb_bytes; c.b_inv_scale = d_b_inv_scale;
  c.C = d_C; c.ldc = ldc; c.accumulate = accumulate;
  c.out_sp = d_out_sp; c.ld_out_sp_bytes = ld_out_sp_bytes; c.out_inv_scale = d_out_inv_scale;
  c.bias = d_bias; c.act = act;
  c.mul = d_mul; c.ld_mul = ld_mul; c.act_of_saved = act_of_saved; c.saved = d_saved; c.ld_saved = ld_saved;
  c.saved_scale = saved_scale; c.dropout_rate = dropout_rate; c.dropout_seed = dropout_seed;
  c.tile_kmask = d_tile_kmask; c.row_map = d_row_map;
  return sp_nt_enqueue(c, (hipStream_t)stream);
}

int tfgnn_sp_gemm_nt_grouped(int64_t M, int64_t N, int64_t K, const void* d_A_sp, int64_t lda_bytes, const float* d_a_inv_scale,
                             int a_scale_block, const int32_t* d_a_rows, int64_t a_src_rows, const int32_t* d_tile_table,
                             int64_t num_tiles, int num_groups, const void* d_B_sp, int64_t ldb_bytes, int64_t b_group_stride_bytes,
                             const float* d_b_inv_scale, int64_t b_scale_group_stride, float* d_C, int64_t ldc, const float* d_bias,
                             int act, const float* d_mul, int64_t ld_mul, int act_of_saved, const float* d_saved, int64_t ld_saved,
                             void* d_out_sp, int64_t ld_out_sp_bytes, float* d_out_inv_scale, void* stream) {
  TFGNN_REQUIRE(d_tile_table && num_tiles > 0 && num_groups >= 1, "tfgnn_sp_gemm_nt_grouped: tile table missing");
  NtCall c;
  c.M = M; c.N = N; c.K = K;
  c.A = d_A_sp; c.lda_bytes = lda_bytes; c.a_inv_scale = d_a_inv_scale; c.a_scale_block = a_scale_block;
  c.a_rows = d_a_rows; c.a_src_rows = a_src_rows;
  c.B = d_B_sp; c.ldb_bytes = ldb_bytes; c.b_inv_scale = d_b_inv_scale;
  c.b_group_stride_bytes = b_group_stride_bytes; c.b_scale_group_stride = b_scale_group_stride;
  c.C = d_C; c.ldc = ldc;
  c.out_sp = d_out_sp; c.ld_out_sp_bytes = ld_out_sp_bytes; c.out_inv_scale = d_out_inv_scale;
  c.bias = d_bias; c.act = act;
  c.mul = d_mul; c.ld_mul = ld_mul; c.act_of_saved = act_of_saved; c.saved = d_saved; c.ld_saved = ld_saved;
  c.tile_table = d_tile_table; c.num_tiles_m = num_tiles; c.num_groups = num_groups;
  return sp_nt_enqueue(c, (hipStream_t)stream);
}

static int64_t sp_tn_plain_ranges(int64_t Mp, int64_t N, int64_t K, int bn, bool wide) {
  const int64_t splits = sp_tn_splits(Mp, N, K, bn);
  return wide ? std::max<int64_t>(splits, ceil_div(K, SP_TN_BSC_MAX_CHUNK)) : splits;
}

static size_t sp_gemm_tn_ws_bytes(int64_t M, int64_t N, int64_t K, int64_t a_total_cols, int a_scale_block, bool wide) {
  const int bn = sp_tile_width(N);
  if (!bn || M <= 0 || a_scale_block <= 0) return 0;
  const int64_t Mp = ceil_div(M, SP_BM) * SP_BM;
  return sp_tn_layout(Mp, N, ceil_div(a_total_cols, a_scale_block), (K + 15) & ~15ll, true, sp_tn_plain_ranges(Mp, N, K, bn, wide),
                      tn_repair_armed() ? kTnRepairTailBytes : 0).total;
}

size_t tfgnn_sp_gemm_tn_workspace_bytes(int64_t M, int64_t N, int64_t K, int64_t a_total_cols, int a_scale_block) {
  return sp_gemm_tn_ws_bytes(M, N, K, a_total_cols, a_scale_block, false);
}

size_t tfgnn_sp_gemm_tn_wide_workspace_bytes(int64_t M, int64_t N, int64_t K, int64_t a_total_cols, int a_scale_block) {
  return sp_gemm_tn_ws_bytes(M, N, K, a_total_cols, a_scale_block, true);
}

static int sp_gemm_tn_plain(bool wide, int64_t M, int64_t N, int64_t K, const void* d_A_sp, int64_t lda_bytes, int64_t a_first_col,
                            const float* d_a_inv_scale, int64_t a_total_cols, int a_scale_block, const void* d_B_sp,
                            int64_t ldb_bytes, int64_t b_first_col, const float* d_b_inv_scale, float* d_C, int64_t group_rows,
                            int64_t stride_group, int64_t stride_row, int64_t stride_col, int accumulate, void* d_workspace,
                            size_t workspace_bytes, void* stream) {
  TFGNN_REQUIRE(d_A_sp && d_B_sp && d_C && d_a_inv_scale, "tfgnn_sp_gemm_tn: null pointer");
  TFGNN_REQUIRE(M > 0 && N > 0 && K > 0, "tfgnn_sp_gemm_tn: empty product");
  if (int rc = sp_tn_check_operands("tfgnn_sp_gemm_tn", M, N, d_A_sp, lda_bytes, a_first_col, a_total_cols, a_scale_block, d_B_sp,
                                    ldb_bytes, b_first_col, true))
    return rc;
  TFGNN_REQUIRE(group_rows > 0, "tfgnn_sp_gemm_tn: group_rows must be positive");
  TFGNN_REQUIRE(a_scale_block >= 48 || a_first_col % a_scale_block == 0,
                "tfgnn_sp_gemm_tn: 32-column scale blocks need a block-aligned first column (at most 4 blocks per 128-column tile)");
  const int64_t Mp = ceil_div(M, SP_BM) * SP_BM;
  const int64_t splits = sp_tn_plain_ranges(Mp, N, K, sp_tile_width(N), wide);
  TFGNN_REQUIRE(!wide || (splits <= kSpTnMaxRanges && d_b_inv_scale),
                "tfgnn_sp_gemm_tn_wide: K too large (more than 512 ranges of 2016 rows), or no scales of B");
  const int64_t nblk = a_total_cols / a_scale_block, kpad = (K + 15) & ~15ll;
  TnLaunch t{};
  t.repair = tn_repair_armed();
  t.lay = sp_tn_layout(Mp, N, nblk, kpad, true, splits, t.repair ? kTnRepairTailBytes : 0);
  if (int rc = sp_tn_check_workspace("tfgnn_sp_gemm_tn", d_workspace, workspace_bytes, t.lay.total)) return rc;
  t.ws = (uint8_t*)d_workspace;
  t.M = M; t.N = N; t.K = K;
  t.A = (const uint8_t*)d_A_sp + a_first_col * 4; t.lda = lda_bytes;
  t.B = (const uint8_t*)d_B_sp + b_first_col * 4; t.ldb = ldb_bytes;
  t.inv_a = d_a_inv_scale; t.inv_b = d_b_inv_scale; t.a_sb = a_scale_block; t.a_col0 = a_first_col; t.a_nblk = (int)nblk;
  t.k_chunk = (((K + 15) / 16 + splits - 1) / splits) * 16;
  t.splits = (int)ceil_div(K, t.k_chunk);
  static const bool fik_env = [] { const char* e = getenv("TFGNN_TN_FIK"); return !e || atoi(e) != 0; }();
  t.form = wide ? TnForm::TwoFactor
                : (fik_env && t.k_chunk <= SP_TN_FIK_MAX_CHUNK && splits <= kSpTnMaxRanges ? TnForm::OneFactor : TnForm::FactorPass);
  TFGNN_REQUIRE(!wide || t.k_chunk <= SP_TN_BSC_MAX_CHUNK, "tfgnn_sp_gemm_tn_wide: K range too long");
  TFGNN_REQUIRE(t.k_chunk * std::max(lda_bytes, ldb_bytes) < (1ll << 31) && nblk * kpad * 2 < (1ll << 31), "tfgnn_sp_gemm_tn: K chunk too large");
  t.C = d_C; t.group_rows = group_rows; t.stride_group = stride_group; t.stride_row = stride_row; t.stride_col = stride_col;
  t.accumulate = accumulate;
  return sp_tn_enqueue(t, (hipStream_t)stream);
}

int tfgnn_sp_gemm_tn(int64_t M, int64_t N, int64_t K, const void* d_A_sp, int64_t lda_bytes, int64_t a_first_col,
                     const float* d_a_inv_scale, int64_t a_total_cols, int a_scale_block, const void* d_B_sp,
                     int64_t ldb_bytes, int64_t b_first_col, const float* d_b_inv_scale, float* d_C, int64_t group_rows,
                     int64_t stride_group, int64_t stride_row, int64_t stride_col, int accumulate, void* d_workspace,
                     size_t workspace_bytes, void* stream) {
  return sp_gemm_tn_plain(false, M, N, K, d_A_sp, lda_bytes, a_first_col, d_a_inv_scale, a_total_cols, a_scale_block, d_B_sp, ldb_bytes,
                          b_first_col, d_b_inv_scale, d_C, group_rows, stride_group, stride_row, stride_col, accumulate, d_workspace,
                          workspace_bytes, stream);
}

int tfgnn_sp_gemm_tn_wide(int64_t M, int64_t N, int64_t K, const void* d_A_sp, int64_t lda_bytes, int64_t a_first_col,
                          const float* d_a_inv_scale, int64_t a_total_cols, int a_scale_block, const void* d_B_sp,
                          int64_t ldb_bytes, int64_t b_first_col, const float* d_b_inv_scale, float* d_C, int64_t group_rows,
                          int64_t stride_group, int64_t stride_row, int64_t stride_col, int accumulate, void* d_workspace,
                          size_t workspace_bytes, void* stream) {
  return sp_gemm_tn_plain(true, M, N, K, d_A_sp, lda_bytes, a_first_col, d_a_inv_scale, a_total_cols, a_scale_block, d_B_sp, ldb_bytes,
                          b_first_col, d_b_inv_scale, d_C, group_rows, stride_group, stride_row, stride_col, accumulate, d_workspace,
                          workspace_bytes, stream);
}

static TnLayout sp_tn_grouped_layout(int64_t M, int64_t N, int64_t nblk, int num_splits) {
  return sp_tn_layout(ceil_div(M, SP_BM) * SP_BM, N, nblk, 0, false, num_splits, tn_repair_armed() ? kTnRepairGroupedTailBytes : 0);
}

size_t tfgnn_sp_gemm_tn_grouped_workspace_bytes(int64_t M, int64_t N, int64_t a_total_cols, int a_scale_block, int num_splits) {
  if (!sp_tile_width(N) || M <= 0 || a_total_cols <= 0 || a_scale_block <= 0 || num_splits < 0) return 0;
  return sp_tn_grouped_layout(M, N, ceil_div(a_total_cols, a_scale_block), num_splits).total;
}

int tfgnn_sp_gemm_tn_grouped(int64_t M, int64_t N, const void* d_A_sp, int64_t lda_bytes, const float* d_a_inv_scale,
                             int64_t a_total_cols, int a_scale_block, const void* d_B_sp, int64_t ldb_bytes, const float* d_b_inv_scale,
                             int num_groups, const int32_t* d_group_split_offsets, int num_splits, const int32_t* d_split_table,
                             float* d_C, int64_t c_group_stride, int64_t stride_row, int64_t stride_col, void* d_workspace,
                             size_t workspace_bytes, void* stream) {
  TFGNN_REQUIRE(d_A_sp && d_B_sp && d_C && d_a_inv_scale && d_b_inv_scale && d_group_split_offsets && d_split_table,
                "tfgnn_sp_gemm_tn_grouped: null pointer");
  TFGNN_REQUIRE(M > 0 && N > 0 && num_groups >= 1 && num_splits >= 0 && num_splits <= kSpTnMaxRanges,
                "tfgnn_sp_gemm_tn_grouped: 1.. groups, at most 512 K ranges");
  if (int rc = sp_tn_check_operands("tfgnn_sp_gemm_tn_grouped", M, N, d_A_sp, lda_bytes, 0, a_total_cols, a_scale_block, d_B_sp, ldb_bytes, 0,
                                    false))
    return rc;
  const int64_t nblk = a_total_cols / a_scale_block;
  TnLaunch t{};
  t.repair = tn_repair_armed();
  t.lay = sp_tn_grouped_layout(M, N, nblk, num_splits);
  if (int rc = sp_tn_check_workspace("tfgnn_sp_gemm_tn_grouped", d_workspace, workspace_bytes, t.lay.total)) return rc;
  t.ws = (uint8_t*)d_workspace;
  t.M = M; t.N = N; t.K = 0;
  t.A = (const uint8_t*)d_A_sp; t.lda = lda_bytes;
  t.B = (const uint8_t*)d_B_sp; t.ldb = ldb_bytes;
  t.inv_a = d_a_inv_scale; t.inv_b = d_b_inv_scale; t.a_sb = a_scale_block; t.a_col0 = 0; t.a_nblk = (int)nblk;
  t.splits = num_splits; t.k_chunk = SP_TN_BSC_MAX_CHUNK; t.split_table = d_split_table;
  t.form = TnForm::TwoFactor;
  t.trip_stride = t.repair ? 1 : 0;
  t.C = d_C; t.group_rows = M; t.stride_row = stride_row; t.stride_col = stride_col;
  t.num_groups = num_groups; t.group_split_offsets = d_group_split_offsets; t.c_group_stride = c_group_stride;
  return sp_tn_enqueue(t, (hipStream_t)stream);
}


int tfgnn_sp_split_rows_job(const float* d_src, int64_t ld, int64_t seg_len, int64_t seg_stride, int64_t rows, int64_t cols,
                            int scale_block, void* d_sp, int64_t ld_sp_bytes, float* d_inv_scale,
                            const float* d_fixed_inv_scale, tfgnn_aux_job* job) {
  TFGNN_REQUIRE(d_src && d_sp && job, "tfgnn_sp_split_rows_job: null pointer");
  TFGNN_REQUIRE(rows > 0 && cols > 0 && cols % 16 == 0, "tfgnn_sp_split_rows_job: cols must be a positive multiple of 16");
  if (scale_block <= 0) scale_block = (int)cols;
  if (seg_len <= 0) { seg_len = cols; seg_stride = 0; }
  TFGNN_REQUIRE(scale_block % 16 == 0 && cols % scale_block == 0, "tfgnn_sp_split_rows_job: scale_block must divide cols and be a multiple of 16");
  TFGNN_REQUIRE(seg_len % 4 == 0 && cols % seg_len == 0 && ld % 4 == 0 && seg_stride % 4 == 0 && (uintptr_t)d_src % 16 == 0,
                "tfgnn_sp_split_rows_job: source must be 16-byte aligned with segment length / strides multiples of 4");
  TFGNN_REQUIRE(ld_sp_bytes >= cols * 4 && ld_sp_bytes % 64 == 0 && (uintptr_t)d_sp % 64 == 0, "tfgnn_sp_split_rows_job: bad SP16 leading dimension / alignment");
  AuxSplitRows a{d_src, ld, seg_len, seg_stride, rows, cols, scale_block, (uint8_t*)d_sp, ld_sp_bytes, d_inv_scale, d_fixed_inv_scale};
  const int64_t items = rows * (cols / scale_block);
  TFGNN_REQUIRE(ceil_div(items, 4) < (1ll << 31), "tfgnn_sp_split_rows_job: too many rows");
  aux_job_set(job, AUX_SPLIT_ROWS, (unsigned)ceil_div(items, 4), a);
  return TFGNN_OK;
}

int tfgnn_sp_split_cols_job(const float* d_src, int64_t ld, int64_t K, int64_t N, void* d_sp, int64_t ld_sp_bytes,
                            float* d_inv_scale, tfgnn_aux_job* job) {
  TFGNN_REQUIRE(d_src && d_sp && job, "tfgnn_sp_split_cols_job: null pointer");
// ... 55 lines not shown
```

tf2_gnn_amd/csrc/gemm_sp.hpp:

```cpp
#pragma once
#include "common.hpp"

namespace tfgnn {

struct NtCall {
  int64_t M = 0, N = 0, K = 0;
  const void* A = nullptr;
  int64_t lda_bytes = 0;
  const float* a_inv_scale = nullptr;
  int a_scale_block = 0;
  const int32_t* a_rows = nullptr;
  int64_t a_src_rows = 0;
  const void* B = nullptr;
  int64_t ldb_bytes = 0;
  const float* b_inv_scale = nullptr;
  int64_t b_group_stride_bytes = -1;
  int64_t b_scale_group_stride = -1;
  float* C = nullptr;
  int64_t ldc = 0;
  int accumulate = 0;
  void* out_sp = nullptr;
  int64_t ld_out_sp_bytes = 0;
  float* out_inv_scale = nullptr;
  const float* bias = nullptr;
  int act = TFGNN_ACT_NONE;
  const float* mul = nullptr;
  int64_t ld_mul = 0;
  int act_of_saved = TFGNN_ACT_NONE;
  const float* saved = nullptr;
  int64_t ld_saved = 0;
  float saved_scale = 1.f;
  float dropout_rate = 0.f;
  uint64_t dropout_seed = 0;
  const uint8_t* tile_kmask = nullptr;
  const int32_t* row_map = nullptr;
  const int32_t* tile_table = nullptr;
  int64_t num_tiles_m = 0;
  int num_groups = 1;
};

int sp_nt_enqueue(const NtCall& c, hipStream_t s);

}
```

tf2_gnn_amd/csrc/mp_layer.hip:

```cpp
#include <cstring>

#include "common.hpp"
#include "gemm_sp.hpp"
#include "tfgnn.h"

using namespace tfgnn;

extern "C" int tfgnn_mp_forward(const tfgnn_mp_forward_args* a, void* stream) {
  TFGNN_REQUIRE(a != nullptr && a->struct_size == sizeof(tfgnn_mp_forward_args),
                "tfgnn_mp_forward: args is NULL or was built against another header (struct_size)");
  TFGNN_REQUIRE(a->kind == TFGNN_MP_AGGREGATE_FIRST, "tfgnn_mp_forward: unknown layer kind %d", a->kind);
  TFGNN_REQUIRE(a->graph && a->x && a->wt_sp && a->wt_inv_scale && a->agg_sp && a->agg_inv_scale && (a->out || a->out_sp),
                "tfgnn_mp_forward: NULL pointer");
  TFGNN_REQUIRE(a->view == TFGNN_VIEW_BY_DST_TYPED || a->view == TFGNN_VIEW_BY_DST_TYPED_PATTERN,
                "tfgnn_mp_forward: the forward pass gathers over the by-target typed buckets (view %d)", a->view);
  int64_t V = 0, E = 0;
  int L = 0;
  int rc = tfgnn_graph_dims(a->graph, &V, &L, &E);
  if (rc) return rc;
  const int64_t D = a->in_dim, H = a->hidden_dim, K = (int64_t)L * D;
  TFGNN_REQUIRE(V > 0 && L > 0 && D > 0 && H > 0, "tfgnn_mp_forward: empty layer");
  rc = tfgnn_graph_gather_reduce_sp(a->graph, a->view, nullptr, nullptr, a->row_scale, a->x, a->ldx, (int)D, a->agg_sp, D * 4,
                                    a->agg_inv_scale, nullptr, a->workspace, a->workspace_bytes, stream);
  if (rc) return rc;
  if (a->w) {
    tfgnn_aux_job job;
    std::memset(&job, 0, sizeof(job));
    rc = tfgnn_sp_split_cols_job(a->w, H, K, H, a->wt_sp, a->ld_wt_sp_bytes, a->wt_inv_scale, &job);
    if (rc) return rc;
    rc = tfgnn_aux_launch(&job, 1, stream);
    if (rc) return rc;
  }
  NtCall c;
  c.M = V; c.N = H; c.K = K;
  c.A = a->agg_sp; c.lda_bytes = K * 4; c.a_inv_scale = a->agg_inv_scale; c.a_scale_block = (int)D;
  c.B = a->wt_sp; c.ldb_bytes = a->ld_wt_sp_bytes; c.b_inv_scale = a->wt_inv_scale;
  c.C = a->out; c.ldc = a->ld_out;
  c.out_sp = a->out_sp; c.ld_out_sp_bytes = a->ld_out_sp_bytes; c.out_inv_scale = a->out_inv_scale;
  c.bias = a->bias; c.act = a->act;
  c.dropout_rate = a->dropout_rate; c.dropout_seed = a->dropout_seed;
  c.tile_kmask = a->tile_kmask; c.row_map = a->row_map;
  return sp_nt_enqueue(c, (hipStream_t)stream);
}

extern "C" int tfgnn_mp_backward(const tfgnn_mp_backward_args* a, void* stream) {
  TFGNN_REQUIRE(a != nullptr && a->struct_size == sizeof(tfgnn_mp_backward_args),
                "tfgnn_mp_backward: args is NULL or was built against another header (struct_size)");
  TFGNN_REQUIRE(a->kind == TFGNN_MP_AGGREGATE_FIRST, "tfgnn_mp_backward: unknown layer kind %d", a->kind);
  TFGNN_REQUIRE(a->graph && a->d_pre && a->wh_sp && a->wh_inv_scale && a->g_sp && a->g_inv_scale && (a->dx || a->dx_sp),
                "tfgnn_mp_backward: NULL pointer");
  TFGNN_REQUIRE(!a->dw || (a->x_sp && a->x_inv_scale), "tfgnn_mp_backward: the kernel gradients need the layer input as a split operand");
  int64_t V = 0, E = 0;
  int L = 0;
  int rc = tfgnn_graph_dims(a->graph, &V, &L, &E);
  if (rc) return rc;
  const int64_t D = a->in_dim, H = a->hidden_dim, K = (int64_t)L * H;
  TFGNN_REQUIRE(V > 0 && L > 0 && D > 0 && H > 0, "tfgnn_mp_backward: empty layer");
  rc = tfgnn_graph_gather_reduce_sp(a->graph, TFGNN_VIEW_BY_SRC_TYPED, nullptr, a->edge_weight, nullptr, a->d_pre, a->ld_d_pre, (int)H,
                                    a->g_sp, H * 4, a->g_inv_scale, nullptr, a->workspace, a->workspace_bytes, stream);
  if (rc) return rc;
  if (a->w) {
    tfgnn_aux_job job;
    std::memset(&job, 0, sizeof(job));
    rc = tfgnn_sp_split_rows_job(a->w, H, H, D * H, D, K, (int)K, a->wh_sp, a->ld_wh_sp_bytes, a->wh_inv_scale, nullptr, &job);
    if (rc) return rc;
    rc = tfgnn_aux_launch(&job, 1, stream);
    if (rc) return rc;
  }
  NtCall c;
  c.M = V; c.N = D; c.K = K;
  c.A = a->g_sp; c.lda_bytes = K * 4; c.a_inv_scale = a->g_inv_scale; c.a_scale_block = (int)H; c.a_rows = a->a_rows;
  c.B = a->wh_sp; c.ldb_bytes = a->ld_wh_sp_bytes; c.b_inv_scale = a->wh_inv_scale;
  c.C = a->dx; c.ldc = a->ld_dx; c.accumulate = a->accumulate;
  c.out_sp = a->dx_sp; c.ld_out_sp_bytes = a->ld_dx_sp_bytes; c.out_inv_scale = a->dx_inv_scale;
  c.mul = a->mul; c.ld_mul = a->ld_mul; c.act_of_saved = a->act_of_saved; c.saved = a->saved; c.ld_saved = a->ld_saved;
  c.saved_scale = a->saved_scale; c.dropout_rate = a->dropout_rate; c.dropout_seed = a->dropout_seed;
  c.tile_kmask = a->tile_kmask; c.row_map = a->row_map;
  rc = sp_nt_enqueue(c, (hipStream_t)stream);
  if (rc) return rc;
  if (a->dw)
    rc = tfgnn_sp_gemm_tn(K, D, V, a->g_sp, K * 4, 0, a->g_inv_scale, K, (int)H, a->x_sp, a->ld_x_sp_bytes, 0, a->x_inv_scale, a->dw, H, D * H, 1,
                          H, 0, a->tn_workspace, a->tn_workspace_bytes, stream);
  return rc;
}
```

tf2_gnn_amd/layers/gnn.py:

```python
from __future__ import annotations

from typing import Any, Dict, List, NamedTuple, Optional, Sequence, Tuple

import torch

from .. import guard, ops
from ..utils.param_helpers import get_activation_function
from .graph_global_exchange import (
    GraphGlobalExchange,
    GraphGlobalExchangeInput,
    GraphGlobalGRUExchange,
    GraphGlobalMeanExchange,
    GraphGlobalMLPExchange,
)
from .message_passing import MessagePassing, MessagePassingInput, get_message_passing_class
from .message_passing.message_passing import Variable, _num_edge_types, default_device, get_graph, glorot_uniform


class GNNInput(NamedTuple):

    node_features: torch.Tensor
    adjacency_lists: Tuple[torch.Tensor, ...]
    node_to_graph_map: torch.Tensor
    num_graphs: Any
# ... 115 lines not shown
                mode = self._params["global_exchange_mode"].lower()
                cls = {"mean": GraphGlobalMeanExchange, "gru": GraphGlobalGRUExchange, "mlp": GraphGlobalMLPExchange}[mode]
                ex = cls(
                    hidden_dim=H,
                    weighting_fun=self._params["global_exchange_weighting_fun"],
                    num_heads=self._params["global_exchange_num_heads"],
                    dropout_rate=self._params["global_exchange_dropout_rate"],
                )
                ex.build(GraphGlobalExchangeInput(embedded_shape, (None,), ()))
                for v in ex.trainable_variables:
                    v.name = f"{name}/Layer_{layer_idx}/Global_Exchange/{v.name}"
                self._global_exchange_layers[str(layer_idx)] = ex
        self.built = True

    def __call__(self, inputs: GNNInput, training: bool = False, return_all_representations: bool = False):
        if not self.built:
            self.build(
                GNNInput(
                    tuple(inputs.node_features.shape),
                    tuple((None, 2) for _ in range(_num_edge_types(inputs.adjacency_lists))),
                    (None,),
                    (),
                )
            )
        return self.call(inputs, training, return_all_representations)

    def call(self, inputs: GNNInput, training: bool = False, return_all_representations: bool = False):
        cur, all_reprs = self._internal_call(inputs, training, need_all_representations=return_all_representations)
        if return_all_representations:
            return cur, all_reprs
        return cur

    def graph_parts(self, num_nodes: int, edges_per_type) -> int:
        if not self._mp_layers:
            return ops.G_PARTS_DEFAULT
        parts = 0
        for mp in self._mp_layers:
            parts |= mp.graph_parts(num_nodes, edges_per_type, self._hidden_dim)
        return parts

    def _dense_f16x2(self, in_dim: int, out_dim: int) -> bool:
        self.guard.sync_with_rearm_epoch()
        if ops.env("TFGNN_DENSE_F16X2", "1") == "0" or self.guard.dense == "exact":
            return False
        return ops.get_gemm_mode() == ops.GEMM_F16X2 and in_dim % 16 == 0 and in_dim >= 32 and ops.sp_tiles(out_dim)

    def _presplit_weights(self, graph, V: int, backward: bool, need_input_grad: bool = False) -> None:
        if V <= 0 or ops.get_gemm_mode() != ops.GEMM_F16X2 or ops.env("TFGNN_PRESPLIT", "1") == "0":
            return
        H = self._hidden_dim
        reqs = []
        dense = [self._initial_projection_layer] + [self._dense_layers[k] for k in sorted(self._dense_layers, key=int)]
        for i, w in enumerate(dense):
            d_in, d_out = w.value.shape
            if not self._dense_f16x2(d_in, d_out):
                continue
            if not backward:
                reqs.append((w.value, "cols", lambda w=w: ops.sp_split_cols_jobs(w.value)))
            elif ops.sp_tiles(d_in) and (i > 0 or need_input_grad):
                reqs.append((w.value, "rows", lambda w=w: ops.sp_split_rows_jobs(w.value)))
        for mp in self._mp_layers:
            reqs.extend(mp.weight_operand_requests(graph, V, H, backward))
        ops.presplit_weight_operands(reqs)

    def _dense(self, x, w: Variable, act_name, drop=None):
        if x.shape[0] > 0 and self._dense_f16x2(w.value.shape[0], w.value.shape[1]):
            wt = ops.sp_weight_operand(w.value, "cols", lambda: ops.sp_split_cols_jobs(w.value))
            if act_name == "gelu":
                pre = ops.sp_gemm_nt(ops.sp_rows_of(x), wt)
                return ops.activation_forward("gelu", pre), pre, False
            if drop is not None and ops.sp_one_tile(w.value.shape[1]):
                out, _ = ops.sp_gemm_nt_split(ops.sp_rows_of(x), wt, act=act_name, dropout=drop)
                return out, None, True
            return ops.sp_gemm_nt(ops.sp_rows_of(x), wt, act=act_name), None, False
        if act_name == "gelu":
            pre = ops.gemm(x, w.value)
            return ops.activation_forward("gelu", pre), pre, False
        return ops.gemm(x, w.value, act=act_name), None, False

    def _dense_backward(self, x, w: Variable, gpre, act_grad=None, need_input_grad=True):
        d_in, d_out = w.value.shape
        if x.shape[0] > 0 and self._dense_f16x2(d_in, d_out):
            g_sp = ops.sp_rows_of(gpre)
            if self.guard.dense == "wide":
                w.grad = ops.sp_gemm_tn(ops.sp_rows_of(x), g_sp, out=torch.empty_like(w.value), wide=True)
            else:
                w.grad = ops.sp_gemm_tn(ops.sp_rows_of(x), g_sp)
            if not need_input_grad:
                return None
            if ops.sp_tiles(d_in):
                wr = ops.sp_weight_operand(w.value, "rows", lambda: ops.sp_split_rows_jobs(w.value))
                return ops.sp_gemm_nt(g_sp, wr, act_grad=act_grad)
            return ops.gemm_grad(gpre, w.value, trans_b=True, act_grad=act_grad)
        w.grad = ops.gemm(x, gpre, trans_a=True)
        return ops.gemm_grad(gpre, w.value, trans_b=True, act_grad=act_grad) if need_input_grad else None

    def _fuse_dropout_statically(self, layer_idx: int) -> bool:
        if ops.get_gemm_mode() != ops.GEMM_F16X2:
            return False
        if layer_idx % self._residual_every_num_layers == 0 and not (layer_idx == 0 and self._residual_every_num_layers >= self._num_layers):
            return False
        if layer_idx == 0:
            return True
        prev = layer_idx - 1
        return not self._use_inter_layer_layernorm and str(prev) not in self._global_exchange_layers

    def _recompute_dropout(self, layer_idx: int, mp_layer, V: int, D: int, L: int) -> bool:
        if ops.env("TFGNN_RECOMPUTE_DROPOUT", "1") == "0" or ops.get_gemm_mode() != ops.GEMM_F16X2:
            return False
        if layer_idx % self._residual_every_num_layers == 0 and not (layer_idx == 0 and self._residual_every_num_layers >= self._num_layers):
            return False
        return bool(getattr(mp_layer, "built", False) and mp_layer.recomputes_input_dropout(V, D, L))

    def _internal_call(self, inputs: GNNInput, training: bool = False, need_all_representations: bool = True):
        X = inputs.node_features
        V = X.shape[0]
        adj = inputs.adjacency_lists
        self.guard.sync_with_rearm_epoch(self._mp_layers)
        graph = adj if isinstance(adj, ops.Graph) else get_graph(
            adj, V, parts=self.graph_parts(V, [int(a.shape[0]) if a.numel() else 0 for a in adj]))
        graph = get_graph(graph, V)
        rate = float(self._params["layer_input_dropout_rate"])
        steps = []
        NL = self._num_layers

        drop_seed, ex_seed = [None] * NL, {}
        for i in range(NL):
            if training and rate > 0.0:
                self._dropout_calls += 1
                drop_seed[i] = self.dropout_seed * 1000003 + self._dropout_calls
            if str(i) in self._global_exchange_layers:
                self._dropout_calls += 1
                ex_seed[i] = self.dropout_seed * 1000003 + self._dropout_calls

        def drop_for(i, producer_output_is_read):
            if i >= NL or drop_seed[i] is None or producer_output_is_read or not self._fuse_dropout_statically(i):
                return None
            return (rate, drop_seed[i])

        self._presplit_weights(graph, V, backward=False)
        cur, pre0, dropped = self._dense(X, self._initial_projection_layer, self._init_act,
                                         drop=drop_for(0, need_all_representations))
        ctx = {"X": X, "graph": graph, "h0": cur, "pre0": pre0, "steps": steps, "h0_scale": (1.0 - rate) if dropped else 1.0,
               "all_representations": need_all_representations}
        last = cur
        all_reprs = [cur]
        for layer_idx, mp_layer in enumerate(self._mp_layers):
            st = {}
            if drop_seed[layer_idx] is not None:
                if dropped:
                    st["drop"] = ops.DropoutSpec(rate, drop_seed[layer_idx], tuple(cur.shape), cur.device)
                    st["drop_by_producer"] = True
                elif self._recompute_dropout(layer_idx, mp_layer, V, int(cur.shape[1]), graph.num_edge_types):
                    st["drop"] = ops.DropoutSpec(rate, drop_seed[layer_idx], tuple(cur.shape), cur.device)
                    cur, _ = ops.dropout_forward(cur, rate, drop_seed[layer_idx], want_mask=False)
                else:
                    cur, st["mask"] = ops.dropout_forward(cur, rate, drop_seed[layer_idx])
            dropped = False
            if layer_idx % self._residual_every_num_layers == 0:
                tmp = cur
                if layer_idx > 0:
                    cur = ops.add_scale(cur, last, 0.5)
                last = tmp
            dense_here = layer_idx % self._dense_every_num_layers == 0
            has_ex = str(layer_idx) in self._global_exchange_layers
            want_split = (dense_here and not has_ex
                          and not self._use_inter_layer_layernorm and self._dense_f16x2(self._hidden_dim, self._hidden_dim))
            direct = not (dense_here or has_ex or self._use_inter_layer_layernorm)
            cur, dropped = mp_layer.call_with_epilogue(
                MessagePassingInput(node_embeddings=cur, adjacency_lists=graph), training=training, want_split_output=want_split,
                output_dropout=drop_for(layer_idx + 1, need_all_representations) if direct else None)
            all_reprs.append(cur)
            if has_ex:
                ex = self._global_exchange_layers[str(layer_idx)]
                ex.dropout_seed = ex_seed[layer_idx]
# ... 143 lines not shown
```

tf2_gnn_amd/ops.py:

```python
from __future__ import annotations

import ctypes
import os
from typing import Dict, Optional, Sequence

import numpy as np
import torch

from . import _lib
from .guard import (
    GEMM_BF16X3, GEMM_BF16X3_EXACT, GEMM_F16X2, GEMM_FP32, capturing, demote_gemm_mode, f16x2_guard_flag_async,
    f16x2_guard_tripped_sync, get_gemm_mode, guard_repair, hold_spread_guard, rearm_spread_guard, repair_stats, set_gemm_mode,
    set_guard_repair)

ACT_NONE, ACT_RELU, ACT_TANH, ACT_LEAKY_RELU, ACT_ELU, ACT_SELU, ACT_GELU, ACT_SIGMOID = range(8)
REDUCE_SUM, REDUCE_MAX = 0, 1

_ACT_BY_NAME = {
    "none": ACT_NONE,
    "relu": ACT_RELU,
    "tanh": ACT_TANH,
    "leaky_relu": ACT_LEAKY_RELU,
    "elu": ACT_ELU,
    "selu": ACT_SELU,
# ... 1520 lines not shown
def sp_gemm_nt_grouped(a: SplitOperand, b: SplitOperand, groups: RowGroups, *, a_rows=None, act=ACT_NONE, act_grad=None,
                       want_fp32: bool = True, want_split: bool = False, b_column_blocks: bool = False):
    lib = _lib.load()
    M, K = groups.num_rows, a.cols
    G = max(groups.num_groups, 1)
    if b_column_blocks:
        if b.cols != G * K or b.scale_block != b.cols:
            raise ValueError("sp_gemm_nt_grouped: b must be [N, G * K] with one scale per row")
        N, stride_b, stride_scale = b.rows, 4 * K, 0
    else:
        if b.cols != K or b.rows % G or b.scale_block != K:
            raise ValueError("sp_gemm_nt_grouped: b must stack one [N, K] operand per group with one scale per row")
        N = b.rows // G
        stride_b, stride_scale = N * b.data.stride(0), N
    if a_rows is None and a.rows != M:
        raise ValueError(f"sp_gemm_nt_grouped: {a.rows} operand rows for {M} grouped rows")
    if a_rows is not None:
        a_rows = _row_map(a_rows, M)
    dev = a.data.device
    out = torch.empty((M, N), dtype=torch.float32, device=dev) if want_fp32 else None
    op = _empty_split(M, N, dev) if want_split else None
    if M == 0:
        return out, op
    _, act_of_saved, saved, _, _, _ = _c_epilogue(None, act_grad, None, 1.0)
    _lib.check(
        lib.tfgnn_sp_gemm_nt_grouped(
            M, N, K, _ptr(a.data), a.data.stride(0), _ptr(a.inv_scale), a.scale_block if a.scale_block else -1, _ptr(a_rows), a.rows,
            _ptr(groups.table), groups.num_tiles, G, _ptr(b.data), b.data.stride(0), stride_b, _ptr(b.inv_scale), stride_scale,
            _ptr(out), N, None, act_id(act), None, 0, act_of_saved, _ptr(saved), saved.stride(0) if saved is not None else 0,
            _ptr(op.data) if op is not None else None, op.data.stride(0) if op is not None else 0,
            _ptr(op.inv_scale) if op is not None else None, _stream(),
        )
    )
    if out is not None and op is not None:
        _remember_split_rows(out, op)
    return out, op


TN_WIDE_MAX_ROWS = 512 * 2016
TN_GROUPED_MAX_RANGES = 512
TN_GROUPED_MAX_CHUNK = 2016


def sp_gemm_tn_grouped(a: SplitOperand, b: SplitOperand, groups: RowGroups, out: torch.Tensor, transposed: bool = False) -> torch.Tensor:
    lib = _lib.load()
    if a.scale_block <= 0 or b.scale_block != b.cols or a.rows != b.rows or a.rows != groups.num_rows:
        raise ValueError("sp_gemm_tn_grouped: operands must share the grouped rows; b needs one scale per row")
    M, N, G = a.cols, b.cols, groups.num_groups
    if not out.is_contiguous() or out.numel() != G * M * N:
        raise ValueError("sp_gemm_tn_grouped: out must be contiguous [G, M, N]")
    tab = groups.tn_tables()
    if tab[2] > TN_GROUPED_MAX_RANGES:
        raise ValueError(f"sp_gemm_tn_grouped: {tab[2]} K ranges, at most {TN_GROUPED_MAX_RANGES} per launch (callers take another route)")
    ws_bytes = lib.tfgnn_sp_gemm_tn_grouped_workspace_bytes(M, N, a.cols, a.scale_block, tab[2])
    ws_ptr, ws_len, _ = _aligned_workspace(a.data.device, ws_bytes)
    sr, sc = (1, M) if transposed else (N, 1)
    _lib.check(lib.tfgnn_sp_gemm_tn_grouped(M, N, _ptr(a.data), a.data.stride(0), _ptr(a.inv_scale), a.cols, a.scale_block, _ptr(b.data),
                                            b.data.stride(0), _ptr(b.inv_scale), G, _ptr(tab[1]), tab[2], _ptr(tab[0]), _ptr(out), M * N, sr, sc,
                                            ctypes.c_void_p(ws_ptr), ws_len, _stream()))
    return out


def sp_gather_rows(a: SplitOperand, index: torch.Tensor) -> SplitOperand:
    lib = _lib.load()
    _require_dev(index, torch.int32, "index")
    n = int(index.numel())
    per = a.inv_scale.shape[1] if a.inv_scale.dim() == 2 else 1
    out = SplitOperand(torch.empty((n, a.cols * 4), dtype=torch.uint8, device=a.data.device),
                       torch.empty((n, per), dtype=torch.float32, device=a.data.device), n, a.cols, a.scale_block)
    _lib.check(lib.tfgnn_sp_gather_rows(_ptr(a.data), a.data.stride(0), _ptr(a.inv_scale), per, _ptr(index.contiguous()), n, a.rows, a.cols,
                                        _ptr(out.data), out.data.stride(0), _ptr(out.inv_scale), _stream()))
    return out


def _nt_shape(who: str, a: SplitOperand, b: SplitOperand):
    M, K, N = a.rows, a.cols, b.rows
    if b.cols != K:
        raise ValueError(f"{who}: inner dimensions differ ({K} vs {b.cols})")
    if b.scale_block != K:
        raise ValueError(f"{who}: the right operand must carry one scale per row")
    return M, K, N


def _sp_gemm_nt_rows(a, b, M, N, K, out, ldc, op, bias, act, accumulate, epilogue, tile_kmask, row_map, a_rows) -> None:
    out_mul, act_of_saved, saved, saved_scale, rate, seed = epilogue
    if bias is not None:
        bias = bias.contiguous()
    _ensure_splitk_workspace(a.data.device, M)
    _lib.check(
        _lib.load().tfgnn_sp_gemm_nt_rows(
            M, N, K, _ptr(a.data), a.data.stride(0), _ptr(a.inv_scale), a.scale_block if a.scale_block else -1,
            _ptr(_row_map(a_rows, M)), _ptr(b.data), b.data.stride(0),
            _ptr(b.inv_scale), _ptr(out), ldc, _ptr(bias), act_id(act), int(accumulate), _ptr(out_mul),
            out_mul.stride(0) if out_mul is not None else 0, act_of_saved, _ptr(saved),
            saved.stride(0) if saved is not None else 0, saved_scale, _ptr(op.data) if op is not None else None,
            op.data.stride(0) if op is not None else 0, _ptr(op.inv_scale) if op is not None else None, rate, seed,
            _ptr(_tile_kmask(tile_kmask, M)), _ptr(_row_map(row_map, M)), _stream(),
        )
    )


@_writes_out
def sp_gemm_nt(a: SplitOperand, b: SplitOperand, *, bias=None, act=ACT_NONE, out=None, accumulate=False, out_mul=None,
               act_grad=None, dropout=None, saved_scale: float = 1.0, tile_kmask=None, row_map=None, a_rows=None) -> torch.Tensor:
    M, K, N = _nt_shape("sp_gemm_nt", a, b)
    out, ldc = _product_out(out, M, N, accumulate, a.data.device)
    _sp_gemm_nt_rows(a, b, M, N, K, out, ldc, None, bias, act, accumulate, _c_epilogue(out_mul, act_grad, dropout, saved_scale),
                     tile_kmask, row_map, a_rows)
    return out


def sp_gemm_nt_split(a: SplitOperand, b: SplitOperand, *, bias=None, act=ACT_NONE, out_mul=None, act_grad=None,
                     want_fp32: bool = True, dropout=None, saved_scale: float = 1.0, tile_kmask=None, row_map=None, a_rows=None):
    M, K, N = _nt_shape("sp_gemm_nt_split", a, b)
    dev = a.data.device
    out = torch.empty((M, N), dtype=torch.float32, device=dev) if want_fp32 else None
    op = _empty_split(M, N, dev)
    _sp_gemm_nt_rows(a, b, M, N, K, out, N, op, bias, act, False, _c_epilogue(out_mul, act_grad, dropout, saved_scale),
                     tile_kmask, row_map, a_rows)
    if out is not None:
        _remember_split_rows(out, op)
    return out, op


def split_rows_remembered(x: torch.Tensor) -> SplitOperand:
    op = sp_split_rows(x)
    _remember_split_rows(x, op)
    return op


def graph_gather_sp(graph: "Graph", view: int, inp: torch.Tensor, *, col=None, edge_weight=None, row_scale=None,
                    fixed_inv_scale: Optional[torch.Tensor] = None, rows_per_operand_row: int = 1) -> SplitOperand:
    lib = _lib.load()
    _require_dev(inp, torch.float32, "inp")
    typed = view in (VIEW_BY_DST_TYPED, VIEW_BY_SRC_TYPED, VIEW_BY_DST_TYPED_PATTERN)
    if view in (VIEW_BY_DST_TYPED_COMPACT, VIEW_BY_SRC_TYPED_COMPACT):
        if rows_per_operand_row != 1:
            raise ValueError("graph_gather_sp: compact rows are operand rows (rows_per_operand_row = 1)")
        num_rows = int(graph.nonempty_offsets(view == VIEW_BY_SRC_TYPED_COMPACT)[-1])
    else:
        num_rows = graph.num_nodes * (graph.num_edge_types if typed else 1)
    if view == VIEW_BY_DST_TYPED_PATTERN and graph.num_edge_types > 8:
        raise ValueError("graph_gather_sp: the pattern order exists for at most 8 edge types")
    inp, ld_in = _rowmajor(inp, "inp")
    width = inp.shape[1]
    R = int(rows_per_operand_row)
    if num_rows % R:
        raise ValueError("rows_per_operand_row must divide the number of rows of the view")
    data = torch.empty((num_rows // R, R * width * 4), dtype=torch.uint8, device=inp.device)
    inv = None
    if fixed_inv_scale is None:
        inv = torch.empty((num_rows // R, R), dtype=torch.float32, device=inp.device)
    graph.ensure(_VIEW_PARTS[view])
    ws_bytes = lib.tfgnn_graph_gather_workspace_bytes(graph._h, view, width)
    ws = _workspace(inp.device, ws_bytes) if ws_bytes else None
    _lib.check(
        lib.tfgnn_graph_gather_reduce_sp(
            graph._h, view, _ptr(col), _ptr(edge_weight), _ptr(row_scale), _ptr(inp), ld_in, width, _ptr(data), width * 4,
            _ptr(inv), _ptr(fixed_inv_scale), _ptr(ws), ws.numel() if ws is not None else 0, _stream(),
        )
    )
    if fixed_inv_scale is not None:
        return SplitOperand(data, fixed_inv_scale, num_rows // R, R * width, 0)
    return SplitOperand(data, inv, num_rows // R, R * width, width)


def mp_entry_enabled() -> bool:
    return env("TFGNN_MP_ENTRY", "1") != "0"


def _weight_operand_for_call(w: torch.Tensor, kind: str, rows: int, cols: int):
    op = _cached_weight_operand(w, kind)
    if op is not None:
        return op, False
    return _empty_split(rows, cols, w.device, per_row=True), True


def mp_forward(graph: "Graph", view: int, x: torch.Tensor, W: torch.Tensor, *, row_scale=None, act=ACT_NONE, dropout=None,
               tile_kmask=None, row_map=None, want_split: bool = False, want_fp32: bool = True):
    lib = _lib.load()
    _require_dev(x, torch.float32, "x")
    L, D, H = (int(v) for v in W.shape)
    V = graph.num_nodes
    if L != graph.num_edge_types or x.shape[1] != D or not W.is_contiguous():
        raise ValueError("mp_forward: W must be the contiguous [L, D, H] stack of the graph's edge types and of x's width")
    x, ldx = _rowmajor(x, "x")
    dev = x.device
    graph.ensure(_VIEW_PARTS[view])
    wt, stale = _weight_operand_for_call(W, "cols", H, L * D)
    agg = torch.empty((V, L * D * 4), dtype=torch.uint8, device=dev)
    agg_inv = torch.empty((V, L), dtype=torch.float32, device=dev)
# ... 63 lines not shown
            tn_ptr, tn_len, tn_ws = _aligned_workspace(dev, tn_bytes, own=True)
    _ensure_splitk_workspace(dev, V)
    stream = _stream()
    skip = skip or {}
    a = _lib.MpBackwardArgs()
    a.struct_size = ctypes.sizeof(_lib.MpBackwardArgs)
    a.kind = 0
    a.graph = graph._h
    a.d_pre, a.ld_d_pre, a.in_dim, a.hidden_dim = d_pre.data_ptr(), ldg, D, H
    a.edge_weight = edge_weight.data_ptr() if edge_weight is not None else None
    a.w = W.data_ptr() if stale else None
    a.wh_sp, a.ld_wh_sp_bytes, a.wh_inv_scale = wh.data.data_ptr(), wh.data.stride(0), wh.inv_scale.data_ptr()
    a.g_sp, a.g_inv_scale = g_sp.data_ptr(), g_inv.data_ptr()
    a.dx, a.ld_dx, a.accumulate = out.data_ptr(), ldc, int(bool(accumulate))
    if out_mul is not None:
        a.mul, a.ld_mul = out_mul.data_ptr(), out_mul.stride(0)
    a.act_of_saved = act_of_saved
    if saved is not None:
        a.saved, a.ld_saved = saved.data_ptr(), saved.stride(0)
    a.saved_scale = saved_scale
    a.dropout_rate, a.dropout_seed = rate, seed
    if op is not None:
        a.dx_sp, a.ld_dx_sp_bytes, a.dx_inv_scale = op.data.data_ptr(), op.data.stride(0), op.inv_scale.data_ptr()
    for name, check in (("tile_kmask", _tile_kmask), ("a_rows", _row_map), ("row_map", _row_map)):
        t = skip.get(name)
        if t is not None:
            setattr(a, name, check(t, V).data_ptr())
    if dW is not None:
        a.dw = dW.data_ptr()
        a.x_sp, a.ld_x_sp_bytes, a.x_inv_scale = x_sp.data.data_ptr(), x_sp.data.stride(0), x_sp.inv_scale.data_ptr()
        a.tn_workspace, a.tn_workspace_bytes = tn_ptr, tn_len
    a.workspace, a.workspace_bytes = (ws.data_ptr(), ws.numel()) if ws is not None else (None, 0)
    _lib.check(lib.tfgnn_mp_backward(ctypes.byref(a), stream))
    if stale:
        _cache_weight_operand(W, "rows", wh)
    del tn_ws
    torch.autograd.graph.increment_version(out)
    if op is not None:
        _remember_split_rows(out, op)
    return out, op, dW


@_writes_out
def sp_gemm_tn(a: SplitOperand, b: SplitOperand, *, a_cols=None, b_cols=None, out: Optional[torch.Tensor] = None,
               scatter=None, accumulate: bool = False, wide: bool = False) -> torch.Tensor:
    lib = _lib.load()
    if a.scale_block <= 0 or b.scale_block != b.cols:
        raise ValueError("sp_gemm_tn: the left operand needs per-(row, block) scales, the right one one scale per row")
    if a.rows != b.rows:
        raise ValueError(f"sp_gemm_tn: K differs ({a.rows} vs {b.rows})")
    if wide and a.rows > TN_WIDE_MAX_ROWS:
        if out is None:
            raise ValueError("sp_gemm_tn(wide=True) over more than %d rows needs out" % TN_WIDE_MAX_ROWS)
        for r0 in range(0, a.rows, TN_WIDE_MAX_ROWS):
            r1 = min(a.rows, r0 + TN_WIDE_MAX_ROWS)
            sp_gemm_tn(SplitOperand(a.data[r0:r1], a.inv_scale[r0:r1], r1 - r0, a.cols, a.scale_block),
                       SplitOperand(b.data[r0:r1], b.inv_scale[r0:r1], r1 - r0, b.cols, b.scale_block),
                       a_cols=a_cols, b_cols=b_cols, out=out, scatter=scatter, accumulate=accumulate or r0 > 0, wide=True)
        return out
    a0, M = a_cols if a_cols is not None else (0, a.cols)
    b0, N = b_cols if b_cols is not None else (0, b.cols)
    K = a.rows
    if out is None:
        if scatter is not None or accumulate:
            raise ValueError("scatter / accumulate need out")
        out = torch.empty((M, N), dtype=torch.float32, device=a.data.device)
    if not out.is_contiguous() or out.numel() != M * N:
        raise ValueError(f"out must be contiguous with {M * N} elements")
    gr, sg, sr, sc = scatter if scatter is not None else (M, 0, N, 1)
    ws_bytes = (lib.tfgnn_sp_gemm_tn_wide_workspace_bytes if wide else lib.tfgnn_sp_gemm_tn_workspace_bytes)(M, N, K, a.cols, a.scale_block)
    ws_ptr, ws_len = None, 0
    if ws_bytes:
        ws_ptr, ws_len, _ = _aligned_workspace(a.data.device, ws_bytes)
        ws_ptr = ctypes.c_void_p(ws_ptr)
    _lib.check(
        (lib.tfgnn_sp_gemm_tn_wide if wide else lib.tfgnn_sp_gemm_tn)(
            M, N, K, _ptr(a.data), a.data.stride(0), a0, _ptr(a.inv_scale), a.cols, a.scale_block, _ptr(b.data),
            b.data.stride(0), b0, _ptr(b.inv_scale), _ptr(out), gr, sg, sr, sc, int(accumulate), ws_ptr, ws_len, _stream(),
        )
    )
    return out


def tensor_inv_scale(bound: torch.Tensor) -> torch.Tensor:
    lib = _lib.load()
    out = torch.empty(1, dtype=torch.float32, device=bound.device)
    _lib.check(lib.tfgnn_sp_inv_scale_from_bound(_ptr(bound.contiguous()), _ptr(out), _stream()))
    return out


def absmax(x: torch.Tensor, scale: float = 1.0) -> torch.Tensor:
    lib = _lib.load()
    _require_dev(x, torch.float32, "x")
    x = x.contiguous()
    out = torch.zeros(1, dtype=torch.float32, device=x.device)
    _lib.check(lib.tfgnn_absmax(_ptr(x), x.numel(), float(scale), _ptr(out), _stream()))
    return out


_sp_weight_cache: "dict" = {}
_CHECK_WEIGHT_CACHE = [None]


def clear_weight_operand_cache() -> None:
    _sp_weight_cache.clear()


def notify_weights_changed(tensor: Optional[torch.Tensor] = None) -> None:
    if tensor is None:
        _sp_weight_cache.clear()
        return
    base = tensor._base if tensor._base is not None else tensor
    lo = base.data_ptr()
    hi = lo + base.numel() * base.element_size()
    for key in [k for k in _sp_weight_cache if lo <= k[0] < hi]:
        del _sp_weight_cache[key]


def _weight_key(w: torch.Tensor, kind: str):
    return (w.data_ptr(), tuple(w.shape), tuple(w.stride()), kind)


def _weight_checksum(w: torch.Tensor):
    if _CHECK_WEIGHT_CACHE[0] is None:
        import os

        _CHECK_WEIGHT_CACHE[0] = os.environ.get("TFGNN_CHECK_WEIGHT_CACHE", "0") == "1"
    if not _CHECK_WEIGHT_CACHE[0]:
        return None
    v = w.detach().double()
    return (float(v.sum()), float(v.abs().sum()))


def sp_weight_operand(w: torch.Tensor, kind: str, build):
    op = _cached_weight_operand(w, kind)
    if op is None:
        op = build()
        if isinstance(op, SplitJobs):
            aux_flush([op])
            op = op.operand
        _cache_weight_operand(w, kind, op)
    return op


def presplit_weight_operands(requests) -> int:
    made, seen = [], set()
    for w, kind, build in requests:
        key = _weight_key(w, kind)
        if key in seen or _cached_weight_operand(w, kind) is not None:
            continue
        seen.add(key)
        made.append((w, kind, build()))
    if made:
        aux_flush([op for _, _, op in made if isinstance(op, SplitJobs)])
        for w, kind, op in made:
            _cache_weight_operand(w, kind, op.operand if isinstance(op, SplitJobs) else op)
    return len(made)


def _cached_weight_operand(w: torch.Tensor, kind: str):
    hit = _sp_weight_cache.get(_weight_key(w, kind))
    if hit is not None and hit[0] == w._version and hit[2]() is not None:
        if hit[3] is not None and hit[3] != _weight_checksum(w):
            raise RuntimeError("a weight tensor changed without a version bump (update through .data or a raw pointer?): "
                               "call Variable.mark_updated() / ops.notify_weights_changed() after such an update")
        return hit[1]
# ... 120 lines not shown
```

Before: 420.3 million edges/s.

## Carry split-K TN weight-grad reduction as tail blocks of the following NT GEMM

The split-K reduction for the weight-gradient TN GEMM used to run as its own kernel. It is now deferred and appended as extra blocks to the grid of the input-gradient NT GEMM that follows. The tail blocks read their arguments from the kernarg segment and run the reduce body, so one launch is removed and the reduce can overlap with the NT tiles. This costs larger kernel arguments, a noinline branch in the hot kernel, a separate owned workspace per TN product, and a check that the TN and NT split-K workspaces do not overlap.

```diff
diff --git a/include/tfgnn.h b/include/tfgnn.h
--- a/include/tfgnn.h
+++ b/include/tfgnn.h
@@ -392,6 +392,25 @@
                      int64_t ldb_bytes, int64_t b_first_col, const float* d_b_inv_scale, float* d_C, int64_t group_rows,
                      int64_t stride_group, int64_t stride_row, int64_t stride_col, int accumulate, void* d_workspace,
                      size_t workspace_bytes, void* stream);
+typedef struct tfgnn_tn_reduce_job {
+  unsigned num_blocks;
+  unsigned reserved;
+  unsigned char payload[184];
+} tfgnn_tn_reduce_job;
+int tfgnn_sp_gemm_tn_product(int64_t M, int64_t N, int64_t K, const void* d_A_sp, int64_t lda_bytes, int64_t a_first_col,
+                              const float* d_a_inv_scale, int64_t a_total_cols, int a_scale_block, const void* d_B_sp,
+                              int64_t ldb_bytes, int64_t b_first_col, const float* d_b_inv_scale, float* d_C, int64_t group_rows,
+                              int64_t stride_group, int64_t stride_row, int64_t stride_col, int accumulate, void* d_workspace,
+                              size_t workspace_bytes, tfgnn_tn_reduce_job* job, void* stream);
+int tfgnn_tn_reduce_launch(const tfgnn_tn_reduce_job* job, void* stream);
+int tfgnn_tn_reduce_counts(int64_t* out_counts, int n);
+int tfgnn_sp_gemm_nt_rows_tail(int64_t M, int64_t N, int64_t K, const void* d_A_sp, int64_t lda_bytes, const float* d_a_inv_scale,
+                               int a_scale_block, const int32_t* d_a_rows, const void* d_B_sp, int64_t ldb_bytes,
+                               const float* d_b_inv_scale, float* d_C, int64_t ldc, const float* d_bias, int act, int accumulate,
+                               const float* d_mul, int64_t ld_mul, int act_of_saved, const float* d_saved, int64_t ld_saved,
+                               float saved_scale, void* d_out_sp, int64_t ld_out_sp_bytes, float* d_out_inv_scale, float dropout_rate,
+                               uint64_t dropout_seed, const uint8_t* d_tile_kmask, const int32_t* d_row_map,
+                               const tfgnn_tn_reduce_job* job, void* stream);
 
 int tfgnn_absmax(const float* d_x, int64_t n, float scale, float* d_out, void* stream);
 int tfgnn_sp_inv_scale_from_bound(const float* d_bound, float* d_inv_scale, void* stream);
diff --git a/tf2_gnn_amd/_lib.py b/tf2_gnn_amd/_lib.py
--- a/tf2_gnn_amd/_lib.py
+++ b/tf2_gnn_amd/_lib.py
@@ -321,6 +321,24 @@
 ]
 
 _SIGNATURES += [
+    (
+        "tfgnn_sp_gemm_tn_product",
+        c_int,
+        [c_int64, c_int64, c_int64, c_void_p, c_int64, c_int64, c_void_p, c_int64, c_int, c_void_p, c_int64, c_int64, c_void_p,
+         c_void_p, c_int64, c_int64, c_int64, c_int64, c_int, c_void_p, c_size_t, c_void_p, c_void_p],
+    ),
+    ("tfgnn_tn_reduce_launch", c_int, [c_void_p, c_void_p]),
+    ("tfgnn_tn_reduce_counts", c_int, [POINTER(c_int64), c_int]),
+    (
+        "tfgnn_sp_gemm_nt_rows_tail",
+        c_int,
+        [c_int64, c_int64, c_int64, c_void_p, c_int64, c_void_p, c_int, c_void_p, c_void_p, c_int64, c_void_p, c_void_p, c_int64,
+         c_void_p, c_int, c_int, c_void_p, c_int64, c_int, c_void_p, c_int64, c_float, c_void_p, c_int64, c_void_p, c_float,
+         ctypes.c_uint64, c_void_p, c_void_p, c_void_p, c_void_p],
+    ),
+]
+
+_SIGNATURES += [
     ("tfgnn_pool_workspace_bytes", c_size_t, [c_int64, c_int64, c_int, c_int, c_int]),
     ("tfgnn_pool_forward", c_int, [c_void_p, c_void_p]),
     ("tfgnn_pool_backward", c_int, [c_void_p, c_void_p]),
@@ -393,6 +411,11 @@
 class AuxJob(ctypes.Structure):
 
     _fields_ = [("kind", c_int), ("num_blocks", ctypes.c_uint), ("payload", ctypes.c_ubyte * 248)]
+
+
+class TnReduceJob(ctypes.Structure):
+
+    _fields_ = [("num_blocks", ctypes.c_uint), ("reserved", ctypes.c_uint), ("payload", ctypes.c_ubyte * 184)]
 
 
 class MpForwardArgs(ctypes.Structure):
diff --git a/tf2_gnn_amd/csrc/gemm_sp.hip b/tf2_gnn_amd/csrc/gemm_sp.hip
--- a/tf2_gnn_amd/csrc/gemm_sp.hip
+++ b/tf2_gnn_amd/csrc/gemm_sp.hip
@@ -1,5 +1,7 @@
 #include <algorithm>
+#include <cstddef>
 #include <cstdlib>
+#include <cstring>
 
 #include <type_traits>
 
@@ -72,6 +74,11 @@
   unsigned xcd_per, xcd_total;
 };
 
+struct SpTail {
+  unsigned first, blocks;
+  TnReduceArgs args;
+};
+
 __global__ void __launch_bounds__(256) sp_split_rows_kernel(const float* __restrict__ src, int64_t ld, int64_t seg_len,
                                                             int64_t seg_stride, int64_t R, int64_t C, int sb,
                                                             uint8_t* __restrict__ dst, int64_t ld_dst, float* __restrict__ inv,
@@ -337,12 +344,67 @@
   }
 };
 
+__device__ __forceinline__ void sp_tn_reduce_body(const TnReduceArgs& a, unsigned block, unsigned nblocks, unsigned nthreads) {
+  const int64_t total = a.M * a.N;
+  for (int64_t i = (int64_t)block * nthreads + threadIdx.x; i < total; i += (int64_t)nblocks * nthreads) {
+    const int64_t m = i / a.N, n = i - m * a.N;
+    const int64_t blk = (a.a_col0 + m) / a.a_sb;
+    float s = 0.f;
+    int z = 0;
+    if (a.ref_ld > 0) {
+      for (; z + 8 <= a.splits; z += 8) {
+        float v[8], r[8];
+#pragma unroll
+        for (int u = 0; u < 8; ++u) {
+          v[u] = a.partial[(int64_t)(z + u) * a.slab + i];
+          r[u] = a.ref[(int64_t)(z + u) * a.ref_ld + blk];
+        }
+#pragma unroll
+        for (int u = 0; u < 8; ++u) s += v[u] * r[u];
+      }
+      for (; z < a.splits; ++z) s += a.partial[(int64_t)z * a.slab + i] * a.ref[(int64_t)z * a.ref_ld + blk];
+    } else {
+      for (; z + 8 <= a.splits; z += 8) {
+        float v[8];
+#pragma unroll
+        for (int u = 0; u < 8; ++u) v[u] = a.partial[(int64_t)(z + u) * a.slab + i];
+#pragma unroll
+        for (int u = 0; u < 8; ++u) s += v[u];
+      }
+      for (; z < a.splits; ++z) s += a.partial[(int64_t)z * a.slab + i];
+      s *= a.ref[blk];
+    }
+    const int64_t gi = m / a.group_rows, mi = m - gi * a.group_rows;
+    float* dst = a.C + gi * a.stride_group + mi * a.stride_row + n * a.stride_col;
+    *dst = a.accumulate ? *dst + s : s;
+  }
+}
+
+__device__ __attribute__((noinline)) void sp_nt_tail_pass(const __attribute__((address_space(4))) unsigned* args, unsigned block,
+                                                          unsigned nblocks, unsigned nthreads) {
+  static_assert(sizeof(SpArgs) % 8 == 0 && offsetof(SpTail, args) % 4 == 0 && sizeof(TnReduceArgs) % 4 == 0, "the pass's arguments are read as dwords");
+  union {
+    TnReduceArgs a;
+    unsigned w[sizeof(TnReduceArgs) / 4];
+  } ta;
+#pragma unroll
+  for (unsigned i = 0; i < sizeof(TnReduceArgs) / 4; ++i) ta.w[i] = (unsigned)__builtin_amdgcn_readfirstlane((int)args[i]);
+  sp_tn_reduce_body(ta.a, (unsigned)__builtin_amdgcn_readfirstlane((int)block), (unsigned)__builtin_amdgcn_readfirstlane((int)nblocks),
+                    (unsigned)__builtin_amdgcn_readfirstlane((int)nthreads));
+}
+
 template <int TNW, bool ABLK, bool GRAD, bool OUT_SP = false>
-__global__ void __launch_bounds__((SpGeo<TNW, sp_nt_tm<TNW>>::NT), (TNW == 2 ? 2 : 1)) gemm_sp_nt_kernel(SpArgs g) {
+__global__ void __launch_bounds__((SpGeo<TNW, sp_nt_tm<TNW>>::NT), (TNW == 2 ? 2 : 1)) gemm_sp_nt_kernel(SpArgs g, SpTail t) {
   constexpr int TM = sp_nt_tm<TNW>;
   using G = SpGeo<TNW, TM>;
   constexpr int WR = 32 * TM;
   extern __shared__ __attribute__((aligned(16))) uint8_t lds[];
+  if (blockIdx.x >= t.first) {
+    sp_nt_tail_pass((const __attribute__((address_space(4))) unsigned*)__builtin_amdgcn_kernarg_segment_ptr() +
+                        (sizeof(SpArgs) + offsetof(SpTail, args)) / 4,
+                    blockIdx.x - t.first, t.blocks, G::NT);
+    return;
+  }
   const int tid = threadIdx.x;
   const int lane = tid & 63;
   const int wave = __builtin_amdgcn_readfirstlane(tid >> 6);
@@ -355,7 +417,7 @@
   int split = 0;
   int S = g.ksplit;
   if (S > 1) {
-    const unsigned nt_all = gridDim.x / (unsigned)S;
+    const unsigned nt_all = t.first / (unsigned)S;
     if (bid < nt_all * (unsigned)(S - 1)) {
       split = 1 + (int)(bid / nt_all);
       bid -= (unsigned)(split - 1) * nt_all;
@@ -1288,57 +1350,7 @@
   store_tile(std::integral_constant<int, 1>{});
 }
 
-struct TnReduceArgs {
-  const float* partial;
-  int splits;
-  int64_t M, N;
-  const float* ref;
-  int64_t a_col0;
-  int a_sb;
-  float* C;
-  int64_t group_rows, stride_group, stride_row, stride_col;
-  int accumulate;
-  int64_t slab;
-  int ref_ld;
-};
-
-__device__ __forceinline__ void sp_tn_reduce_body(const TnReduceArgs& a, unsigned block, unsigned nblocks) {
-  const int64_t total = a.M * a.N;
-  for (int64_t i = (int64_t)block * 256 + threadIdx.x; i < total; i += (int64_t)nblocks * 256) {
-    const int64_t m = i / a.N, n = i - m * a.N;
-    const int64_t blk = (a.a_col0 + m) / a.a_sb;
-    float s = 0.f;
-    int z = 0;
-    if (a.ref_ld > 0) {
-      for (; z + 8 <= a.splits; z += 8) {
-        float v[8], r[8];
-#pragma unroll
-        for (int u = 0; u < 8; ++u) {
-          v[u] = a.partial[(int64_t)(z + u) * a.slab + i];
-          r[u] = a.ref[(int64_t)(z + u) * a.ref_ld + blk];
-        }
-#pragma unroll
-        for (int u = 0; u < 8; ++u) s += v[u] * r[u];
-      }
-      for (; z < a.splits; ++z) s += a.partial[(int64_t)z * a.slab + i] * a.ref[(int64_t)z * a.ref_ld + blk];
-    } else {
-      for (; z + 8 <= a.splits; z += 8) {
-        float v[8];
-#pragma unroll
-        for (int u = 0; u < 8; ++u) v[u] = a.partial[(int64_t)(z + u) * a.slab + i];
-#pragma unroll
-        for (int u = 0; u < 8; ++u) s += v[u];
-      }
-      for (; z < a.splits; ++z) s += a.partial[(int64_t)z * a.slab + i];
-      s *= a.ref[blk];
-    }
-    const int64_t gi = m / a.group_rows, mi = m - gi * a.group_rows;
-    float* dst = a.C + gi * a.stride_group + mi * a.stride_row + n * a.stride_col;
-    *dst = a.accumulate ? *dst + s : s;
-  }
-}
-
-__global__ void __launch_bounds__(256) sp_tn_reduce_kernel(TnReduceArgs a) { sp_tn_reduce_body(a, blockIdx.x, gridDim.x); }
+__global__ void __launch_bounds__(256) sp_tn_reduce_kernel(TnReduceArgs a) { sp_tn_reduce_body(a, blockIdx.x, gridDim.x, 256); }
 __global__ void __launch_bounds__(256) sp_tn_reduce_grouped_kernel(TnReduceArgs a, const int32_t* __restrict__ split_off,
                                                                    int64_t c_group_stride) {
   const int gq = blockIdx.y;
@@ -1347,7 +1359,7 @@
   a.ref += (int64_t)s0 * a.ref_ld;
   a.splits = s1 - s0;
   a.C += (int64_t)gq * c_group_stride;
-  sp_tn_reduce_body(a, blockIdx.x, gridDim.x);
+  sp_tn_reduce_body(a, blockIdx.x, gridDim.x, 256);
 }
 
 static int sp_tn_splits(int64_t M, int64_t N, int64_t K, int bn) {
@@ -1358,7 +1370,7 @@
 }
 
 template <int TNW>
-static void launch_sp_nt(const SpArgs& g_in, dim3 grid, hipStream_t s) {
+static void launch_sp_nt(const SpArgs& g_in, SpTail t, dim3 grid, hipStream_t s) {
   using G = SpGeo<TNW, sp_nt_tm<TNW>>;
   SpArgs g = g_in;
   g.xcd_per = g.xcd_total = 0;
@@ -1368,10 +1380,12 @@
     g.xcd_per = (grid.x + 7u) / 8u;
     grid.x = g.xcd_per * 8u;
   }
+  t.first = grid.x;
+  grid.x += t.blocks;
   const bool ablk = g.a_inv && g.a_nblk > 1;
   const bool grad = g.mul || g.saved;
   count_launch(TFGNN_KFAM_SP_NT);
-  using Kernel = void (*)(SpArgs);
+  using Kernel = void (*)(SpArgs, SpTail);
   static const Kernel kernels[2][2][2] = {
       {{gemm_sp_nt_kernel<TNW, false, false, false>, gemm_sp_nt_kernel<TNW, false, false, true>},
        {gemm_sp_nt_kernel<TNW, false, true, false>, gemm_sp_nt_kernel<TNW, false, true, true>}},
@@ -1384,7 +1398,7 @@
     (void)hipFuncSetAttribute((const void*)kernel, hipFuncAttributeMaxDynamicSharedMemorySize, G::LDS_BYTES);
     attr_set[ablk][grad][out_sp] = true;
   }
-  hipLaunchKernelGGL(kernel, grid, dim3(G::NT), G::LDS_BYTES, s, g);
+  hipLaunchKernelGGL(kernel, grid, dim3(G::NT), G::LDS_BYTES, s, g, t);
 }
 
 constexpr size_t kSplitkFlagBytes = 65536;
@@ -1527,7 +1541,21 @@
   int64_t c_group_stride;
 };
 
-static int sp_tn_enqueue(const TnLaunch& t, hipStream_t s) {
+static int64_t g_tn_reduce_own = 0, g_tn_reduce_carried = 0;
+
+static unsigned sp_nt_tail_blocks(int64_t total) { return (unsigned)std::max<int64_t>(1, std::min<int64_t>(1024, ceil_div(total, 512))); }
+
+static int sp_tn_reduce_launch(const TnReduceArgs& ra, hipStream_t s) {
+  const int64_t rblocks = ceil_div(ra.M * ra.N, 256);
+  hipLaunchKernelGGL(sp_tn_reduce_kernel, dim3((unsigned)std::min<int64_t>(rblocks, 2048)), dim3(256), 0, s, ra);
+  TFGNN_LAUNCH_CHECK();
+  __atomic_fetch_add(&g_tn_reduce_own, 1, __ATOMIC_RELAXED);
+  return TFGNN_OK;
+}
+
+int sp_tn_reduce_enqueue(const TnReduceJob& job, hipStream_t s) { return sp_tn_reduce_launch(job.args, s); }
+
+static int sp_tn_enqueue_product(const TnLaunch& t, hipStream_t s, TnReduceArgs* ra_out) {
   const int bn = sp_tile_width(t.N);
   const int64_t Mp = ceil_div(t.M, SP_BM) * SP_BM;
   const bool armed = t.repair && t.splits > 0, per_split = t.form != TnForm::FactorPass;
@@ -1587,14 +1615,21 @@
   ra.splits = t.group_split_offsets ? 0 : t.splits;
   ra.C = t.C; ra.group_rows = t.group_rows; ra.stride_group = t.stride_group; ra.stride_row = t.stride_row; ra.stride_col = t.stride_col;
   ra.accumulate = t.accumulate; ra.slab = Mp * t.N;
+  *ra_out = ra;
+  return TFGNN_OK;
+}
+
+static bool sp_tn_reduce_can_defer(const TnLaunch& t) { return !t.group_split_offsets && t.splits > 0; }
+
+static int sp_tn_enqueue(const TnLaunch& t, hipStream_t s) {
+  TnReduceArgs ra{};
+  if (int rc = sp_tn_enqueue_product(t, s, &ra)) return rc;
+  if (!t.group_split_offsets) return sp_tn_reduce_launch(ra, s);
   const int64_t rblocks = ceil_div(t.M * t.N, 256);
-  if (t.group_split_offsets) {
-    hipLaunchKernelGGL(sp_tn_reduce_grouped_kernel, dim3((unsigned)std::min<int64_t>(rblocks, 512), (unsigned)t.num_groups), dim3(256), 0, s,
-                       ra, t.group_split_offsets, t.c_group_stride);
-  } else {
-    hipLaunchKernelGGL(sp_tn_reduce_kernel, dim3((unsigned)std::min<int64_t>(rblocks, 2048)), dim3(256), 0, s, ra);
-  }
+  hipLaunchKernelGGL(sp_tn_reduce_grouped_kernel, dim3((unsigned)std::min<int64_t>(rblocks, 512), (unsigned)t.num_groups), dim3(256), 0, s,
+                     ra, t.group_split_offsets, t.c_group_stride);
   TFGNN_LAUNCH_CHECK();
+  __atomic_fetch_add(&g_tn_reduce_own, 1, __ATOMIC_RELAXED);
   return TFGNN_OK;
 }
 
@@ -1733,16 +1768,29 @@
 }
 
 int sp_nt_enqueue(const NtCall& c, hipStream_t s) {
+  const TnReduceJob* tail = (c.tail && c.tail->blocks) ? c.tail : nullptr;
+  if (tail) {
+    const uintptr_t t0 = (uintptr_t)tail->ws, t1 = t0 + tail->ws_bytes, k0 = (uintptr_t)g_splitk.base, k1 = k0 + g_splitk.bytes;
+    TFGNN_REQUIRE(!(g_splitk.base && t0 < k1 && k0 < t1),
+                  "tfgnn_sp_gemm_nt: the workspace of the carried TN reduction overlaps the K-split workspace of the NT product");
+    if (c.M == 0) return sp_tn_reduce_enqueue(*tail, s);
+  }
   NtShape d;
   int rc = sp_nt_check(c, &d);
   if (rc) return rc;
   SpArgs g = sp_nt_args(c, d);
   rc = sp_nt_plan_splitk(g, d, s);
   if (rc) return rc;
-  const dim3 grid((unsigned)(d.tiles * g.ksplit));
-  if (d.bn == 320) launch_sp_nt<5>(g, grid, s);
-  else if (d.bn == 256) launch_sp_nt<4>(g, grid, s);
-  else launch_sp_nt<2>(g, grid, s);
+  dim3 grid((unsigned)(d.tiles * g.ksplit));
+  SpTail t{};
+  if (tail) {
+    t.args = tail->args;
+    t.blocks = tail->blocks;
+    __atomic_fetch_add(&g_tn_reduce_carried, 1, __ATOMIC_RELAXED);
+  }
+  if (d.bn == 320) launch_sp_nt<5>(g, t, grid, s);
+  else if (d.bn == 256) launch_sp_nt<4>(g, t, grid, s);
+  else launch_sp_nt<2>(g, t, grid, s);
   TFGNN_LAUNCH_CHECK();
   return TFGNN_OK;
 }
@@ -1956,7 +2004,7 @@
                             const float* d_a_inv_scale, int64_t a_total_cols, int a_scale_block, const void* d_B_sp,
                             int64_t ldb_bytes, int64_t b_first_col, const float* d_b_inv_scale, float* d_C, int64_t group_rows,
                             int64_t stride_group, int64_t stride_row, int64_t stride_col, int accumulate, void* d_workspace,
-                            size_t workspace_bytes, void* stream) {
+                            size_t workspace_bytes, void* stream, TnReduceJob* job = nullptr) {
   TFGNN_REQUIRE(d_A_sp && d_B_sp && d_C && d_a_inv_scale, "tfgnn_sp_gemm_tn: null pointer");
   TFGNN_REQUIRE(M > 0 && N > 0 && K > 0, "tfgnn_sp_gemm_tn: empty product");
   if (int rc = sp_tn_check_operands("tfgnn_sp_gemm_tn", M, N, d_A_sp, lda_bytes, a_first_col, a_total_cols, a_scale_block, d_B_sp,
@@ -1988,7 +2036,90 @@
   TFGNN_REQUIRE(t.k_chunk * std::max(lda_bytes, ldb_bytes) < (1ll << 31) && nblk * kpad * 2 < (1ll << 31), "tfgnn_sp_gemm_tn: K chunk too large");
   t.C = d_C; t.group_rows = group_rows; t.stride_group = stride_group; t.stride_row = stride_row; t.stride_col = stride_col;
   t.accumulate = accumulate;
-  return sp_tn_enqueue(t, (hipStream_t)stream);
+  if (!job) return sp_tn_enqueue(t, (hipStream_t)stream);
+  *job = TnReduceJob{};
+  if (!sp_tn_reduce_can_defer(t)) return sp_tn_enqueue(t, (hipStream_t)stream);
+  if (int rc = sp_tn_enqueue_product(t, (hipStream_t)stream, &job->args)) return rc;
+  job->blocks = sp_nt_tail_blocks(M * N);
+  job->ws = d_workspace;
+  job->ws_bytes = t.lay.total;
+  return TFGNN_OK;
+}
+
+}
+
+namespace tfgnn {
+int sp_gemm_tn_product(int64_t M, int64_t N, int64_t K, const void* d_A_sp, int64_t lda_bytes, int64_t a_first_col,
+                        const float* d_a_inv_scale, int64_t a_total_cols, int a_scale_block, const void* d_B_sp, int64_t ldb_bytes,
+                        int64_t b_first_col, const float* d_b_inv_scale, float* d_C, int64_t group_rows, int64_t stride_group,
+                        int64_t stride_row, int64_t stride_col, int accumulate, void* d_workspace, size_t workspace_bytes,
+                        TnReduceJob* job, hipStream_t s) {
+  TFGNN_REQUIRE(job, "tfgnn_sp_gemm_tn_product: null job");
+  return sp_gemm_tn_plain(false, M, N, K, d_A_sp, lda_bytes, a_first_col, d_a_inv_scale, a_total_cols, a_scale_block, d_B_sp, ldb_bytes,
+                          b_first_col, d_b_inv_scale, d_C, group_rows, stride_group, stride_row, stride_col, accumulate, d_workspace,
+                          workspace_bytes, (void*)s, job);
+}
+}
+
+extern "C" {
+
+static_assert(sizeof(tfgnn_tn_reduce_job) >= sizeof(TnReduceJob) && offsetof(TnReduceJob, blocks) == 0,
+              "tfgnn_tn_reduce_job holds a TnReduceJob, the workgroup count first");
+
+int tfgnn_sp_gemm_tn_product(int64_t M, int64_t N, int64_t K, const void* d_A_sp, int64_t lda_bytes, int64_t a_first_col,
+                              const float* d_a_inv_scale, int64_t a_total_cols, int a_scale_block, const void* d_B_sp,
+                              int64_t ldb_bytes, int64_t b_first_col, const float* d_b_inv_scale, float* d_C, int64_t group_rows,
+                              int64_t stride_group, int64_t stride_row, int64_t stride_col, int accumulate, void* d_workspace,
+                              size_t workspace_bytes, tfgnn_tn_reduce_job* job, void* stream) {
+  TFGNN_REQUIRE(job, "tfgnn_sp_gemm_tn_product: null job");
+  TnReduceJob j{};
+  std::memset(job, 0, sizeof(*job));
+  if (int rc = sp_gemm_tn_product(M, N, K, d_A_sp, lda_bytes, a_first_col, d_a_inv_scale, a_total_cols, a_scale_block, d_B_sp, ldb_bytes,
+                                   b_first_col, d_b_inv_scale, d_C, group_rows, stride_group, stride_row, stride_col, accumulate,
+                                   d_workspace, workspace_bytes, &j, (hipStream_t)stream))
+    return rc;
+  std::memcpy(job, &j, sizeof(j));
+  return TFGNN_OK;
+}
+
+int tfgnn_tn_reduce_launch(const tfgnn_tn_reduce_job* job, void* stream) {
+  TFGNN_REQUIRE(job, "tfgnn_tn_reduce_launch: null job");
+  TnReduceJob j;
+  std::memcpy(&j, job, sizeof(j));
+  if (!j.blocks) return TFGNN_OK;
+  return sp_tn_reduce_enqueue(j, (hipStream_t)stream);
+}
+
+int tfgnn_tn_reduce_counts(int64_t* out_counts, int n) {
+  TFGNN_REQUIRE(out_counts && n >= 0, "tfgnn_tn_reduce_counts: bad argument");
+  const int64_t v[2] = {__atomic_load_n(&g_tn_reduce_own, __ATOMIC_RELAXED), __atomic_load_n(&g_tn_reduce_carried, __ATOMIC_RELAXED)};
+  for (int i = 0; i < n; ++i) out_counts[i] = i < 2 ? v[i] : 0;
+  return TFGNN_OK;
+}
+
+int tfgnn_sp_gemm_nt_rows_tail(int64_t M, int64_t N, int64_t K, const void* d_A_sp, int64_t lda_bytes, const float* d_a_inv_scale,
+                               int a_scale_block, const int32_t* d_a_rows, const void* d_B_sp, int64_t ldb_bytes,
+                               const float* d_b_inv_scale, float* d_C, int64_t ldc, const float* d_bias, int act, int accumulate,
+                               const float* d_mul, int64_t ld_mul, int act_of_saved, const float* d_saved, int64_t ld_saved,
+                               float saved_scale, void* d_out_sp, int64_t ld_out_sp_bytes, float* d_out_inv_scale, float dropout_rate,
+                               uint64_t dropout_seed, const uint8_t* d_tile_kmask, const int32_t* d_row_map,
+                               const tfgnn_tn_reduce_job* job, void* stream) {
+  NtCall c;
+  c.M = M; c.N = N; c.K = K;
+  c.A = d_A_sp; c.lda_bytes = lda_bytes; c.a_inv_scale = d_a_inv_scale; c.a_scale_block = a_scale_block; c.a_rows = d_a_rows;
+  c.B = d_B_sp; c.ldb_bytes = ldb_bytes; c.b_inv_scale = d_b_inv_scale;
+  c.C = d_C; c.ldc = ldc; c.accumulate = accumulate;
+  c.out_sp = d_out_sp; c.ld_out_sp_bytes = ld_out_sp_bytes; c.out_inv_scale = d_out_inv_scale;
+  c.bias = d_bias; c.act = act;
+  c.mul = d_mul; c.ld_mul = ld_mul; c.act_of_saved = act_of_saved; c.saved = d_saved; c.ld_saved = ld_saved;
+  c.saved_scale = saved_scale; c.dropout_rate = dropout_rate; c.dropout_seed = dropout_seed;
+  c.tile_kmask = d_tile_kmask; c.row_map = d_row_map;
+  TnReduceJob j{};
+  if (job) {
+    std::memcpy(&j, job, sizeof(j));
+    c.tail = &j;
+  }
+  return sp_nt_enqueue(c, (hipStream_t)stream);
 }
 
 int tfgnn_sp_gemm_tn(int64_t M, int64_t N, int64_t K, const void* d_A_sp, int64_t lda_bytes, int64_t a_first_col,
diff --git a/tf2_gnn_amd/csrc/gemm_sp.hpp b/tf2_gnn_amd/csrc/gemm_sp.hpp
--- a/tf2_gnn_amd/csrc/gemm_sp.hpp
+++ b/tf2_gnn_amd/csrc/gemm_sp.hpp
@@ -2,6 +2,27 @@
 #include "common.hpp"
 
 namespace tfgnn {
+
+struct TnReduceArgs {
+  const float* partial;
+  int splits;
+  int64_t M, N;
+  const float* ref;
+  int64_t a_col0;
+  int a_sb;
+  float* C;
+  int64_t group_rows, stride_group, stride_row, stride_col;
+  int accumulate;
+  int64_t slab;
+  int ref_ld;
+};
+
+struct TnReduceJob {
+  unsigned blocks;
+  TnReduceArgs args;
+  const void* ws;
+  size_t ws_bytes;
+};
 
 struct NtCall {
   int64_t M = 0, N = 0, K = 0;
@@ -37,8 +58,17 @@
   const int32_t* tile_table = nullptr;
   int64_t num_tiles_m = 0;
   int num_groups = 1;
+  const TnReduceJob* tail = nullptr;
 };
 
 int sp_nt_enqueue(const NtCall& c, hipStream_t s);
 
+int sp_tn_reduce_enqueue(const TnReduceJob& job, hipStream_t s);
+
+int sp_gemm_tn_product(int64_t M, int64_t N, int64_t K, const void* d_A_sp, int64_t lda_bytes, int64_t a_first_col,
+                        const float* d_a_inv_scale, int64_t a_total_cols, int a_scale_block, const void* d_B_sp, int64_t ldb_bytes,
+                        int64_t b_first_col, const float* d_b_inv_scale, float* d_C, int64_t group_rows, int64_t stride_group,
+                        int64_t stride_row, int64_t stride_col, int accumulate, void* d_workspace, size_t workspace_bytes,
+                        TnReduceJob* job, hipStream_t s);
+
 }
diff --git a/tf2_gnn_amd/csrc/mp_layer.hip b/tf2_gnn_amd/csrc/mp_layer.hip
--- a/tf2_gnn_amd/csrc/mp_layer.hip
+++ b/tf2_gnn_amd/csrc/mp_layer.hip
@@ -5,6 +5,8 @@
 #include "tfgnn.h"
 
 using namespace tfgnn;
+
+constexpr int64_t kCarryMaxRowTiles = 4 * 256;
 
 extern "C" int tfgnn_mp_forward(const tfgnn_mp_forward_args* a, void* stream) {
   TFGNN_REQUIRE(a != nullptr && a->struct_size == sizeof(tfgnn_mp_forward_args),
@@ -67,6 +69,16 @@
     rc = tfgnn_aux_launch(&job, 1, stream);
     if (rc) return rc;
   }
+  const bool carry = a->dw && (V + 127) / 128 <= kCarryMaxRowTiles;
+  TnReduceJob reduce{};
+  if (carry) {
+    const uintptr_t t0 = (uintptr_t)a->tn_workspace, t1 = t0 + a->tn_workspace_bytes;
+    const uintptr_t w0 = (uintptr_t)a->workspace, w1 = w0 + a->workspace_bytes;
+    TFGNN_REQUIRE(!(a->tn_workspace && a->workspace && t0 < w1 && w0 < t1), "tfgnn_mp_backward: tn_workspace overlaps workspace");
+    rc = sp_gemm_tn_product(K, D, V, a->g_sp, K * 4, 0, a->g_inv_scale, K, (int)H, a->x_sp, a->ld_x_sp_bytes, 0, a->x_inv_scale, a->dw, H,
+                            D * H, 1, H, 0, a->tn_workspace, a->tn_workspace_bytes, &reduce, (hipStream_t)stream);
+    if (rc) return rc;
+  }
   NtCall c;
   c.M = V; c.N = D; c.K = K;
   c.A = a->g_sp; c.lda_bytes = K * 4; c.a_inv_scale = a->g_inv_scale; c.a_scale_block = (int)H; c.a_rows = a->a_rows;
@@ -76,10 +88,10 @@
   c.mul = a->mul; c.ld_mul = a->ld_mul; c.act_of_saved = a->act_of_saved; c.saved = a->saved; c.ld_saved = a->ld_saved;
   c.saved_scale = a->saved_scale; c.dropout_rate = a->dropout_rate; c.dropout_seed = a->dropout_seed;
   c.tile_kmask = a->tile_kmask; c.row_map = a->row_map;
+  c.tail = &reduce;
   rc = sp_nt_enqueue(c, (hipStream_t)stream);
-  if (rc) return rc;
-  if (a->dw)
-    rc = tfgnn_sp_gemm_tn(K, D, V, a->g_sp, K * 4, 0, a->g_inv_scale, K, (int)H, a->x_sp, a->ld_x_sp_bytes, 0, a->x_inv_scale, a->dw, H, D * H, 1,
+  if (rc && reduce.blocks) (void)sp_tn_reduce_enqueue(reduce, (hipStream_t)stream);
+  if (rc || !a->dw || carry) return rc;
+  return tfgnn_sp_gemm_tn(K, D, V, a->g_sp, K * 4, 0, a->g_inv_scale, K, (int)H, a->x_sp, a->ld_x_sp_bytes, 0, a->x_inv_scale, a->dw, H, D * H, 1,
                           H, 0, a->tn_workspace, a->tn_workspace_bytes, stream);
-  return rc;
 }
diff --git a/tf2_gnn_amd/layers/gnn.py b/tf2_gnn_amd/layers/gnn.py
--- a/tf2_gnn_amd/layers/gnn.py
+++ b/tf2_gnn_amd/layers/gnn.py
@@ -221,15 +221,19 @@
         d_in, d_out = w.value.shape
         if x.shape[0] > 0 and self._dense_f16x2(d_in, d_out):
             g_sp = ops.sp_rows_of(gpre)
+            nt_follows = need_input_grad and ops.sp_tiles(d_in)
+            job = None
             if self.guard.dense == "wide":
                 w.grad = ops.sp_gemm_tn(ops.sp_rows_of(x), g_sp, out=torch.empty_like(w.value), wide=True)
+            elif nt_follows:
+                w.grad, job = ops.sp_gemm_tn_product(ops.sp_rows_of(x), g_sp)
             else:
                 w.grad = ops.sp_gemm_tn(ops.sp_rows_of(x), g_sp)
             if not need_input_grad:
                 return None
-            if ops.sp_tiles(d_in):
+            if nt_follows:
                 wr = ops.sp_weight_operand(w.value, "rows", lambda: ops.sp_split_rows_jobs(w.value))
-                return ops.sp_gemm_nt(g_sp, wr, act_grad=act_grad)
+                return ops.sp_gemm_nt(g_sp, wr, act_grad=act_grad, tail=job)
             return ops.gemm_grad(gpre, w.value, trans_b=True, act_grad=act_grad)
         w.grad = ops.gemm(x, gpre, trans_a=True)
         return ops.gemm_grad(gpre, w.value, trans_b=True, act_grad=act_grad) if need_input_grad else None
diff --git a/tf2_gnn_amd/ops.py b/tf2_gnn_amd/ops.py
--- a/tf2_gnn_amd/ops.py
+++ b/tf2_gnn_amd/ops.py
@@ -1626,31 +1626,71 @@
     return M, K, N
 
 
-def _sp_gemm_nt_rows(a, b, M, N, K, out, ldc, op, bias, act, accumulate, epilogue, tile_kmask, row_map, a_rows) -> None:
+def _sp_gemm_nt_rows(a, b, M, N, K, out, ldc, op, bias, act, accumulate, epilogue, tile_kmask, row_map, a_rows, tail=None) -> None:
     out_mul, act_of_saved, saved, saved_scale, rate, seed = epilogue
     if bias is not None:
         bias = bias.contiguous()
     _ensure_splitk_workspace(a.data.device, M)
-    _lib.check(
-        _lib.load().tfgnn_sp_gemm_nt_rows(
-            M, N, K, _ptr(a.data), a.data.stride(0), _ptr(a.inv_scale), a.scale_block if a.scale_block else -1,
-            _ptr(_row_map(a_rows, M)), _ptr(b.data), b.data.stride(0),
-            _ptr(b.inv_scale), _ptr(out), ldc, _ptr(bias), act_id(act), int(accumulate), _ptr(out_mul),
-            out_mul.stride(0) if out_mul is not None else 0, act_of_saved, _ptr(saved),
-            saved.stride(0) if saved is not None else 0, saved_scale, _ptr(op.data) if op is not None else None,
-            op.data.stride(0) if op is not None else 0, _ptr(op.inv_scale) if op is not None else None, rate, seed,
-            _ptr(_tile_kmask(tile_kmask, M)), _ptr(_row_map(row_map, M)), _stream(),
-        )
+    args = (
+        M, N, K, _ptr(a.data), a.data.stride(0), _ptr(a.inv_scale), a.scale_block if a.scale_block else -1,
+        _ptr(_row_map(a_rows, M)), _ptr(b.data), b.data.stride(0),
+        _ptr(b.inv_scale), _ptr(out), ldc, _ptr(bias), act_id(act), int(accumulate), _ptr(out_mul),
+        out_mul.stride(0) if out_mul is not None else 0, act_of_saved, _ptr(saved),
+        saved.stride(0) if saved is not None else 0, saved_scale, _ptr(op.data) if op is not None else None,
+        op.data.stride(0) if op is not None else 0, _ptr(op.inv_scale) if op is not None else None, rate, seed,
+        _ptr(_tile_kmask(tile_kmask, M)), _ptr(_row_map(row_map, M)),
     )
+    if tail is None:
+        _lib.check(_lib.load().tfgnn_sp_gemm_nt_rows(*args, _stream()))
+        return
+    _lib.check(_lib.load().tfgnn_sp_gemm_nt_rows_tail(*args, ctypes.byref(tail._take()), _stream()))
+    tail._issued()
+
+
+class TnReduceJob:
+
+    def __init__(self, c_job, out: torch.Tensor, workspace):
+        self._c, self.out, self._ws, self._done = c_job, out, workspace, False
+
+    @property
+    def num_blocks(self) -> int:
+        return int(self._c.num_blocks)
+
+    @num_blocks.setter
+    def num_blocks(self, n: int) -> None:
+        if self._c.num_blocks and n > 0:
+            self._c.num_blocks = int(n)
+
+    def _take(self):
+        if self._done:
+            raise RuntimeError("TnReduceJob: the reduce pass has been issued already")
+        return self._c
+
+    def _issued(self) -> None:
+        self._done, self._ws = True, None
+        torch.autograd.graph.increment_version(self.out)
+
+
+def tn_reduce_launch(job: TnReduceJob) -> torch.Tensor:
+    _lib.check(_lib.load().tfgnn_tn_reduce_launch(ctypes.byref(job._take()), _stream()))
+    job._issued()
+    return job.out
+
+
+def tn_reduce_counts() -> dict:
+    buf = (ctypes.c_int64 * 2)()
+    _lib.check(_lib.load().tfgnn_tn_reduce_counts(buf, 2))
+    return {"own": int(buf[0]), "carried": int(buf[1])}
 
 
 @_writes_out
 def sp_gemm_nt(a: SplitOperand, b: SplitOperand, *, bias=None, act=ACT_NONE, out=None, accumulate=False, out_mul=None,
-               act_grad=None, dropout=None, saved_scale: float = 1.0, tile_kmask=None, row_map=None, a_rows=None) -> torch.Tensor:
+               act_grad=None, dropout=None, saved_scale: float = 1.0, tile_kmask=None, row_map=None, a_rows=None,
+               tail: Optional["TnReduceJob"] = None) -> torch.Tensor:
     M, K, N = _nt_shape("sp_gemm_nt", a, b)
     out, ldc = _product_out(out, M, N, accumulate, a.data.device)
     _sp_gemm_nt_rows(a, b, M, N, K, out, ldc, None, bias, act, accumulate, _c_epilogue(out_mul, act_grad, dropout, saved_scale),
-                     tile_kmask, row_map, a_rows)
+                     tile_kmask, row_map, a_rows, tail)
     return out
 
 
@@ -1880,6 +1920,39 @@
     return out
 
 
+def sp_gemm_tn_product(a: SplitOperand, b: SplitOperand, *, a_cols=None, b_cols=None, out: Optional[torch.Tensor] = None,
+                        scatter=None, accumulate: bool = False):
+    lib = _lib.load()
+    if a.scale_block <= 0 or b.scale_block != b.cols:
+        raise ValueError("sp_gemm_tn: the left operand needs per-(row, block) scales, the right one one scale per row")
+    if a.rows != b.rows:
+        raise ValueError(f"sp_gemm_tn: K differs ({a.rows} vs {b.rows})")
+    a0, M = a_cols if a_cols is not None else (0, a.cols)
+    b0, N = b_cols if b_cols is not None else (0, b.cols)
+    K = a.rows
+    if out is None:
+        if scatter is not None or accumulate:
+            raise ValueError("scatter / accumulate need out")
+        out = torch.empty((M, N), dtype=torch.float32, device=a.data.device)
+    if not out.is_contiguous() or out.numel() != M * N:
+        raise ValueError(f"out must be contiguous with {M * N} elements")
+    gr, sg, sr, sc = scatter if scatter is not None else (M, 0, N, 1)
+    ws_bytes = lib.tfgnn_sp_gemm_tn_workspace_bytes(M, N, K, a.cols, a.scale_block)
+    ws_ptr, ws_len, ws = None, 0, None
+    if ws_bytes:
+        ws_ptr, ws_len, ws = _aligned_workspace(a.data.device, ws_bytes, own=True)
+        ws_ptr = ctypes.c_void_p(ws_ptr)
+    c_job = _lib.TnReduceJob()
+    _lib.check(
+        lib.tfgnn_sp_gemm_tn_product(
+            M, N, K, _ptr(a.data), a.data.stride(0), a0, _ptr(a.inv_scale), a.cols, a.scale_block, _ptr(b.data),
+            b.data.stride(0), b0, _ptr(b.inv_scale), _ptr(out), gr, sg, sr, sc, int(accumulate), ws_ptr, ws_len,
+            ctypes.byref(c_job), _stream(),
+        )
+    )
+    return out, TnReduceJob(c_job, out, ws)
+
+
 def tensor_inv_scale(bound: torch.Tensor) -> torch.Tensor:
     lib = _lib.load()
     out = torch.empty(1, dtype=torch.float32, device=bound.device)
```

Measured after the change: 431.6 million edges/s (median of 6 runs). +2.7%, better.
